# ounben/fishnet

Measured on AMD Instinct MI355X. Metric: NNUE evals/sec (node) at 1/2/4/8 MI355X + FT gather HBM GB/s as % of peak, higher is better.
Workload: dtype int16/int8

## Files before the change

fishnet_amd/csrc/gpu_nnue.hip:

```cpp
#include <stdarg.h>
#include <stdio.h>
#include <string.h>

#include <algorithm>
#include <atomic>
#include <chrono>
#include <condition_variable>
#include <memory>
#include <mutex>
#include <string>
#include <thread>
#include <vector>

#include "archive.h"
#include "host_board.h"
#include "kernels.h"
#include "sha256.h"

using namespace gn;

static thread_local std::string g_err;

static int fail(int code, const char *fmt, ...) {
  char buf[512];
// ... 116 lines not shown
    if (!r.u32(hs) || hs != ah) return fail(GN_E_FORMAT, "bad layer-stack hash in stack %d", s);
    bool ok = true;
    for (int i = 0; i < 16 && ok; ++i) ok = r.u32(reinterpret_cast<uint32_t &>(h.b0[s * 16 + i]));
    ok = ok && r.take(&h.w0[(size_t)s * 16 * l1], (size_t)16 * l1);
    for (int i = 0; i < 32 && ok; ++i) ok = r.u32(reinterpret_cast<uint32_t &>(h.b1[s * 32 + i]));
    ok = ok && r.take(&h.w1[s * 1024], 1024);
    ok = ok && r.u32(reinterpret_cast<uint32_t &>(h.b2[s]));
    ok = ok && r.take(&h.w2[s * 32], 32);
    if (!ok) return fail(GN_E_FORMAT, "truncated layer stack %d", s);
  }
  if (r.off != len) return fail(GN_E_FORMAT, "%zu trailing bytes after the network", len - r.off);
  return GN_OK;
}

template <class T>
struct DevBuf {
  T *p = nullptr;
  size_t cap = 0;
  hipError_t ensure(size_t n) {
    if (n <= cap) return hipSuccess;
    const size_t want = std::max(n, cap + cap / 2);
    if (p) (void)hipFree(p);
    p = nullptr;
    cap = 0;
    hipError_t e = hipMalloc(&p, (std::max<size_t>(want, 1) * sizeof(T) + 15) & ~(size_t)15);
    if (e == hipSuccess) cap = want;
    return e;
  }
  void release() {
    if (p) (void)hipFree(p);
    p = nullptr, cap = 0;
  }
};

struct EvalBufs {
  DevBuf<int2> osm, obg;
  DevBuf<uint8_t> nsm, nbg;
  void release() { osm.release(), obg.release(), nsm.release(), nbg.release(); }
};

constexpr size_t FAST_NB0 = 128, FAST_MAX = 4096;
struct FastBatch {
  size_t nb = 0, c1 = 0, c2 = 0;
  int mode = -1;
  uint64_t gen = 0;
  hipGraph_t graph = nullptr;
  hipGraphExec_t exec = nullptr;
  hipEvent_t done = nullptr;
  bool busy = false;
  gn_board *h_in = nullptr;
  gn_eval *h_out = nullptr;
  DevBuf<gn_board> all;
  DevBuf<gn_eval> rec;
  gn_board *in = nullptr, *r1 = nullptr, *r2 = nullptr;
  gn_eval *out = nullptr, *e1 = nullptr, *e2 = nullptr;
  DevBuf<uint64_t> off0, off1;
  DevBuf<uint16_t> m1, m2;
  DevBuf<int32_t> sv1, sv2;
  EvalBufs eb;
  ~FastBatch() {
    if (done) (void)hipEventDestroy(done);
    if (exec) (void)hipGraphExecDestroy(exec);
    if (graph) (void)hipGraphDestroy(graph);
    if (h_in) (void)hipHostFree(h_in);
    if (h_out) (void)hipHostFree(h_out);
    all.release(), rec.release();
    off0.release(), off1.release(), m1.release(), m2.release(), sv1.release(), sv2.release();
    eb.release();
  }
};

struct ExpSet {
  DevBuf<uint64_t> counts, offsets;
  DevBuf<uint32_t> owner;
  DevBuf<Board> unpacked;
  DevBuf<uint16_t> moves_tmp;
  const uint16_t *child_moves = nullptr;
  DevBuf<int2> pinfo;
  DevBuf<int2> p_osm, p_obg;
  DevBuf<uint8_t> p_nsm, p_nbg;
  EvalBufs eb;
  DevBuf<gn_board> children;
  int chain_k = 1;
  int slices = 1;
  bool planned = false;
  uint64_t etot = 0;
  void *scan_tmp = nullptr, *sort_tmp = nullptr;
  size_t scan_bytes = 0, sort_bytes = 0;
  hipEvent_t scored = nullptr;
  DevBuf<uint32_t> perr;
  DevBuf<unsigned long long> pstat;
  DevBuf<uint64_t> ent, eoff;
  DevBuf<TileDesc> tiles;
  DevBuf<uint32_t> btiles, border;
  void release() {
    perr.release(), pstat.release();
    ent.release(), eoff.release(), tiles.release(), btiles.release(), border.release();
    counts.release(), offsets.release(), owner.release(), unpacked.release(), moves_tmp.release();
    pinfo.release(), p_osm.release(), p_obg.release(), p_nsm.release(), p_nbg.release(), eb.release();
    children.release();
    if (scan_tmp) (void)hipFree(scan_tmp);
    if (sort_tmp) (void)hipFree(sort_tmp);
    scan_tmp = sort_tmp = nullptr, scan_bytes = sort_bytes = 0;
    if (scored) (void)hipEventDestroy(scored);
    scored = nullptr;
  }
};

struct Dev {
  int id = 0;
  hipStream_t stream = nullptr;
  void *net_mem[2] = {nullptr, nullptr};
  NetDevice net[2] = {};
  bool has[2] = {false, false};
  Tables *tables = nullptr;
  ExpSet cur, alt;
  DevBuf<gn_board> io_boards, frontier;
  DevBuf<gn_eval> io_out, io_out2;
  DevBuf<uint32_t> off32;
  DevBuf<uint16_t> moves;
  DevBuf<ChildDelta> deltas;
  DevBuf<uint64_t> kkeys, kkeys2;
  DevBuf<uint32_t> kidx, kperm;
  DevBuf<unsigned long long> sum;
  DevBuf<uint8_t> nslot;
  DevBuf<int32_t> part;
  bool part_locked = false;
  DevBuf<uint64_t> ebound;
  DevBuf<uint32_t> pool;
  DevBuf<uint16_t> bkeys, bkeys2;
  DevBuf<uint32_t> bidx;
  hipEvent_t done = nullptr;
  hipStream_t done_on = nullptr;
  float plan_ms = 0, stream_ms = 0, finish_ms = 0;
  struct ScoreLevel {
    DevBuf<uint64_t> sel, pos, counts, offsets;
    DevBuf<uint32_t> idx, owner;
    DevBuf<gn_board> boards, children;
    DevBuf<uint16_t> moves;
    DevBuf<gn_eval> ce;
    DevBuf<int32_t> sv;
    void release() {
      sel.release(), pos.release(), counts.release(), offsets.release(), idx.release(), owner.release();
      boards.release(), children.release(), moves.release(), ce.release(), sv.release();
    }
  } lv[2];
  hipStream_t copy = nullptr;
  hipEvent_t cev[2] = {nullptr, nullptr};
  DevBuf<gn_eval> po2[2], co2[2];
  DevBuf<gn_child> cc2[2];
  DevBuf<uint16_t> mv2[2];
  DevBuf<gn_board> roots, rboards, par;
  DevBuf<uint64_t> moff;
  DevBuf<uint16_t> codes, smoves;
  DevBuf<int32_t> rstatus;
  DevBuf<uint32_t> gidx;
  double t_upload = 0, t_replay = 0, t_compute = 0, t_download = 0, t_tail = 0;
  std::unique_ptr<FastBatch> fast[6][3][2];
  std::condition_variable fast_cv;
  hipStream_t front = nullptr;
  hipEvent_t ev_streamed = nullptr, ev_planned = nullptr;
  std::mutex mu;
};

static void swap_sets(Dev &d) { std::swap(d.cur, d.alt); }

static hipError_t seq_begin(Dev &d, hipStream_t s) {
  if (d.done_on && d.done_on != s) return hipStreamWaitEvent(s, d.done, 0);
  return hipSuccess;
}
static hipError_t seq_end(Dev &d, hipStream_t s) {
  hipError_t e = hipEventRecord(d.done, s);
  if (e == hipSuccess) d.done_on = s;
  return e;
}
static int check_plan(Dev &d, hipStream_t s) {
  if (!d.cur.planned || !d.cur.perr.p) return GN_OK;
  uint32_t e = 0;
  HIP_TRY(hipMemcpyAsync(&e, d.cur.perr.p, sizeof(e), hipMemcpyDeviceToHost, s));
  HIP_TRY(hipStreamSynchronize(s));
  if (e) return fail(GN_E_HIP, "planned expansion failed on the device (error bits 0x%x)", e);
  return GN_OK;
}

struct SeqGuard {
  Dev &d;
  hipStream_t s;
  hipError_t e;
  bool ended = false;
  SeqGuard(Dev &d_, hipStream_t s_) : d(d_), s(s_) { e = seq_begin(d, s); }
  hipError_t finish() {
    ended = true;
    hipError_t r = seq_end(d, s);
    return r == hipSuccess ? hipStreamSynchronize(s) : r;
  }
  ~SeqGuard() {
    if (!ended) (void)seq_end(d, s);
  }
};

#ifndef GN_MAX_LEADERS
#define GN_MAX_LEADERS 1
#endif
constexpr int MAX_LEADERS = GN_MAX_LEADERS;
struct BatchReq {
  const gn_board *boards;
  size_t n;
  int mode;
  gn_eval *out;
  int rc = GN_OK;
  bool done = false;
  bool taken = false;
  char err[256] = "";
};

struct gn_ctx {
  std::vector<std::unique_ptr<Dev>> devs;
  struct {
    std::mutex mu;
    std::condition_variable cv;
    std::vector<BatchReq *> q;
    int active = 0;
    uint64_t launches = 0, calls = 0;
  } co;
  bool coalesce = true;
  bool fast_batch = true;
  int pipeline = 2;
  std::atomic<uint64_t> graph_gen{0};
  std::atomic<uint64_t> fast_runs{0}, fast_fallbacks{0};
  gn_eval_params P;
  bool incremental = true;
  int swizzle = 9;
  int king_sort = 1;
  int chain = 81;
  bool king_cache = true;
  int stream_slices = 3;
  int64_t chunk_parents = 0;
  int l1[2] = {0, 0};
  uint32_t hash[2] = {0, 0};
  double t_parse = 0, t_total = 0;
};

enum { BIG = 0, SMALL = 1 };

static gn_eval_params default_params() {
  gn_eval_params P;
  P.small_net_threshold = 962;
  P.psqt_weight = 125;
  P.positional_weight = 131;
  P.reeval_threshold = 236;
  P.complexity_div_small = 18000;
  P.complexity_div_big = 18000;
  P.material_pawn_small = 535;
  P.material_pawn_big = 535;
  P.material_base = 77777;
  P.rule50_div = 212;
  P.value_clamp = 31506;
  const int32_t pv[5] = {208, 781, 825, 1276, 2538};
  memcpy(P.piece_value, pv, sizeof(pv));
  const double wa[4] = {-37.45051876, 121.19101539, -132.78783573, 420.70576692};
  memcpy(P.wdl_a, wa, sizeof(wa));
  P.wdl_material_min = 17;
  P.wdl_material_max = 78;
  P.wdl_material_anchor = 58;
  const int32_t ww[5] = {1, 3, 3, 5, 9};
  memcpy(P.wdl_piece_weight, ww, sizeof(ww));
  return P;
}

static size_t align256(size_t x) { return (x + 255) & ~(size_t)255; }

static int upload_net(Dev &d, int which, const HostNet &h) {
  const size_t RS = ft_row_stride((uint32_t)h.L1);
  size_t off[10], o = 0;
  const int carry = h.L1 == 128 ? 0 : CARRY_SLOTS;
  std::vector<int32_t> psqt((size_t)PSQT_BUCKETS * FT_ROWS);
  for (size_t r = 0; r < (size_t)FT_ROWS; ++r)
    for (int b = 0; b < PSQT_BUCKETS; ++b)
      memcpy(&psqt[(size_t)b * FT_ROWS + r], h.ft.data() + r * RS + 2 * (size_t)h.L1 + 4 * b, 4);
  const int KS = h.L1 / 64;
  std::vector<int8_t> w0f(h.w0.size());
  for (int b = 0; b < LAYER_STACKS; ++b)
    for (int ks = 0; ks < KS; ++ks)
      for (int ln = 0; ln < 64; ++ln)
        memcpy(&w0f[(((size_t)b * KS + ks) * 64 + ln) * 16],
               &h.w0[((size_t)b * 16 + (ln & 15)) * h.L1 + 64 * (size_t)ks + 16 * (ln >> 4)], 16);
  const size_t sz[10] = {((size_t)FT_ROWS + 4 * (size_t)carry + 128 * (size_t)carry + (carry ? 1 : 0)) * RS, h.bias.size() * 2, h.w0.size(), h.b0.size() * 4,
                         h.w1.size(), h.b1.size() * 4, h.w2.size(), h.b2.size() * 4, psqt.size() * 4, w0f.size()};
  const void *src[10] = {h.ft.data(), h.bias.data(), h.w0.data(), h.b0.data(),
                         h.w1.data(), h.b1.data(), h.w2.data(), h.b2.data(), psqt.data(), w0f.data()};
  for (int i = 0; i < 10; ++i) off[i] = o, o += align256(sz[i]);
  uint8_t *m = nullptr;
  if (hipMalloc(&m, o) != hipSuccess) return fail(GN_E_NOMEM, "device allocation of %zu bytes failed", o);
  d.net_mem[which] = m;
  for (int i = 0; i < 10; ++i)
    HIP_TRY(hipMemcpy(m + off[i], src[i], i == 0 ? (size_t)FT_ROWS * RS : sz[i], hipMemcpyHostToDevice));
  if (carry) HIP_TRY(hipMemset(m + off[0] + (size_t)FT_ROWS * RS, 0, 4 * (size_t)carry * RS));
  if (carry) HIP_TRY(hipMemset(m + off[0] + (size_t)ZERO_ROW * RS, 0, RS));
  NetDevice &n = d.net[which];
  n.L1 = h.L1;
  n.row_stride = (uint32_t)RS;
  n.carry_slots = carry;
  n.kc_slots = carry;
  n.ft = m + off[0];
  n.bias = reinterpret_cast<const int16_t *>(m + off[1]);
  n.w0 = reinterpret_cast<const int8_t *>(m + off[2]);
  n.b0 = reinterpret_cast<const int32_t *>(m + off[3]);
  n.w1 = reinterpret_cast<const int8_t *>(m + off[4]);
  n.b1 = reinterpret_cast<const int32_t *>(m + off[5]);
  n.w2 = reinterpret_cast<const int8_t *>(m + off[6]);
  n.b2 = reinterpret_cast<const int32_t *>(m + off[7]);
  n.psqt = reinterpret_cast<const int32_t *>(m + off[8]);
  n.w0f = reinterpret_cast<const int8_t *>(m + off[9]);
  d.has[which] = true;
  return GN_OK;
}

static void destroy(gn_ctx *ctx) {
  if (!ctx) return;
  for (auto &dp : ctx->devs) {
    Dev &d = *dp;
    (void)hipSetDevice(d.id);
    if (d.stream) (void)hipStreamSynchronize(d.stream);
    for (void *m : d.net_mem)
      if (m) (void)hipFree(m);
    if (d.tables) (void)hipFree(d.tables);
    d.cur.release(), d.alt.release();
    d.io_boards.release(), d.frontier.release(), d.io_out.release(), d.io_out2.release();
    d.off32.release(), d.moves.release(), d.sum.release(), d.deltas.release();
    d.part.release();
    if (d.front) (void)hipStreamSynchronize(d.front), (void)hipStreamDestroy(d.front);
    if (d.ev_streamed) (void)hipEventDestroy(d.ev_streamed);
    if (d.ev_planned) (void)hipEventDestroy(d.ev_planned);
    d.kkeys.release(), d.kkeys2.release(), d.kidx.release(), d.kperm.release();
    d.nslot.release();
    d.ebound.release(), d.pool.release();
    d.bkeys.release(), d.bkeys2.release(), d.bidx.release();
    d.lv[0].release(), d.lv[1].release();
    for (auto &row : d.fast)
      for (auto &pair : row)
        for (auto &f : pair) f.reset();
    for (int i = 0; i < 2; ++i) {
      d.po2[i].release(), d.co2[i].release(), d.cc2[i].release(), d.mv2[i].release();
      if (d.cev[i]) (void)hipEventDestroy(d.cev[i]);
    }
    d.roots.release(), d.rboards.release(), d.par.release(), d.moff.release(), d.codes.release();
    d.smoves.release(), d.rstatus.release(), d.gidx.release();
    if (d.copy) (void)hipStreamSynchronize(d.copy), (void)hipStreamDestroy(d.copy);
    if (d.done) (void)hipEventDestroy(d.done);
    if (d.stream) (void)hipStreamDestroy(d.stream);
  }
  delete ctx;
}

static int create(const uint8_t *big, size_t big_len, const uint8_t *small, size_t small_len, const int *devices,
                  int n_devices, gn_ctx **out) {
  if (!out) return fail(GN_E_INVALID, "out is NULL");
  *out = nullptr;
  if (!big && !small) return fail(GN_E_INVALID, "no network given");
  HostNet hn[2];
  if (big) {
    int rc = parse_net(big, big_len, hn[BIG]);
    if (rc) return rc;
  }
  if (small) {
    int rc = parse_net(small, small_len, hn[SMALL]);
    if (rc) return rc;
  }
  int count = 0;
  if (hipGetDeviceCount(&count) != hipSuccess || count <= 0) return fail(GN_E_NODEVICE, "no HIP device visible");
  std::vector<int> ids;
  if (devices && n_devices > 0) ids.assign(devices, devices + n_devices);
  else ids.push_back(0);
  std::unique_ptr<gn_ctx, void (*)(gn_ctx *)> ctx(new gn_ctx(), destroy);
  ctx->P = default_params();
  for (int w = 0; w < 2; ++w) ctx->l1[w] = hn[w].L1, ctx->hash[w] = hn[w].hash;
  for (int id : ids) {
    if (id < 0 || id >= count) return fail(GN_E_NODEVICE, "device %d out of range (%d visible)", id, count);
    hipDeviceProp_t prop;
    HIP_TRY(hipGetDeviceProperties(&prop, id));
    if (!strstr(prop.gcnArchName, "gfx950"))
      return fail(GN_E_NODEVICE, "device %d is %s; libgpu_nnue is built for gfx950 only", id, prop.gcnArchName);
    ctx->devs.emplace_back(new Dev());
    Dev &d = *ctx->devs.back();
    d.id = id;
    HIP_TRY(hipSetDevice(id));
    HIP_TRY(hipStreamCreateWithFlags(&d.stream, hipStreamNonBlocking));
    HIP_TRY(hipEventCreateWithFlags(&d.done, hipEventDisableTiming));
    HIP_TRY(hipStreamCreateWithFlags(&d.copy, hipStreamNonBlocking));
#ifdef GN_AB_FRONT_PRIORITY
    {
      int least = 0, greatest = 0;
      HIP_TRY(hipDeviceGetStreamPriorityRange(&least, &greatest));
      HIP_TRY(hipStreamCreateWithPriority(&d.front, hipStreamNonBlocking, greatest));
    }
#else
    HIP_TRY(hipStreamCreateWithFlags(&d.front, hipStreamNonBlocking));
#endif
    HIP_TRY(hipEventCreateWithFlags(&d.ev_streamed, hipEventDisableTiming));
    HIP_TRY(hipEventCreateWithFlags(&d.ev_planned, hipEventDisableTiming));
    for (int i = 0; i < 2; ++i) HIP_TRY(hipEventCreateWithFlags(&d.cev[i], hipEventDisableTiming));
#ifdef GN_AB_AUX_STREAMS
    {
      hipStream_t x[2];
      for (int i = 0; i < 2; ++i) HIP_TRY(hipStreamCreateWithFlags(&x[i], hipStreamNonBlocking));
    }
#endif
    HIP_TRY(hipMalloc(&d.tables, sizeof(Tables)));
    for (ExpSet *x : {&d.cur, &d.alt}) {
      HIP_TRY(x->perr.ensure(1));
      HIP_TRY(x->pstat.ensure(1));
      HIP_TRY(hipEventCreateWithFlags(&x->scored, hipEventDisableTiming));
    }
    HIP_TRY(hipMemset(d.alt.perr.p, 0, sizeof(uint32_t)));
    HIP_TRY(hipMemcpy(d.tables, &host_tables(), sizeof(Tables), hipMemcpyHostToDevice));
    for (int w = 0; w < 2; ++w)
      if (hn[w].L1) {
        int rc = upload_net(d, w, hn[w]);
        if (rc) return rc;
      }
// ... 61 lines not shown
                            mode == GN_MODE_FULL ? &P : nullptr, nsm.p, nbg.p));
  HIP_TRY(mark(2));
  if (mode != GN_MODE_SMALL)
    HIP_TRY(launch_eval_net(d.net[BIG], b, mode == GN_MODE_FULL ? nbg.p : nullptr, n, obg.p, perm, swz, s,
                            rows_out));
  HIP_TRY(mark(3));
  HIP_TRY(launch_finalize(b, n, mode, osm.p, obg.p, nsm.p, nbg.p, P, d.tables, out, s, score, counts));
  HIP_TRY(mark(4));
  return GN_OK;
}

static Dev *slot(gn_ctx *ctx, int s) {
  if (!ctx || s < 0 || s >= (int)ctx->devs.size()) return nullptr;
  return ctx->devs[s].get();
}

template <class F>
static void parallel_for(size_t n, size_t grain, F &&f) {
  unsigned hw = std::max(1u, std::min(16u, std::thread::hardware_concurrency()));
  size_t chunks = std::min<size_t>(hw, (n + grain - 1) / std::max<size_t>(grain, 1));
  if (chunks <= 1) {
    f(0, n);
    return;
  }
  std::vector<std::thread> th;
  size_t per = (n + chunks - 1) / chunks;
  for (size_t c = 0; c < chunks; ++c) {
    size_t lo = c * per, hi = std::min(n, lo + per);
    if (lo < hi) th.emplace_back([=, &f] { f(lo, hi); });
  }
  for (auto &t : th) t.join();
}

static int chain_len(const gn_ctx *ctx, Dev &d, size_t n) {
  if (!ctx->incremental || (ctx->chain >= -1 && ctx->chain <= 1) || !d.has[BIG] || !d.net[BIG].carry_slots)
    return 1;
  if (ctx->chain < 0) return -ctx->chain;
  size_t k = (size_t)ctx->chain;
  if ((n + k - 1) / k < 2048) k = std::max<size_t>(2, std::min(k, n / 2048));
  return (int)k;
}

static bool plan_path(const gn_ctx *ctx, const Dev &d, int mode) {
  return mode != GN_MODE_SMALL && ctx->incremental && d.has[BIG] &&
         (d.net[BIG].L1 == 3072 || d.net[BIG].L1 == 1024);
}

static int finalize_all(gn_ctx *ctx, Dev &d, const gn_board *parents, const gn_board *children, int mode,
                        gn_eval *parent_out, gn_eval *child_out, size_t n, size_t total, hipStream_t s,
                        bool score_parents, bool sliced = false) {
  const gn_eval_params &P = ctx->P;
  const ExpSet &x = d.cur;
  const SlicedOut sc = {&d.net[BIG], d.part.p, x.pinfo.p, (uint64_t)(n + total), (uint64_t)n},
                  sp = {&d.net[BIG], d.part.p, x.pinfo.p, (uint64_t)(n + total), 0};
  const bool fast = x.child_moves != nullptr;
  HIP_TRY(launch_finalize(children, total, mode, x.eb.osm.p, x.eb.obg.p, x.eb.nsm.p, x.eb.nbg.p, P, d.tables, child_out,
                          s, 0, nullptr, fast ? x.owner.p : nullptr, fast ? x.child_moves : nullptr,
                          fast ? x.unpacked.p : nullptr, sliced ? &sc : nullptr));
  if (parent_out)
    HIP_TRY(launch_finalize(parents, n, mode, x.p_osm.p, x.p_obg.p, x.p_nsm.p, x.p_nbg.p, P, d.tables, parent_out, s,
                            score_parents ? 1 : 0, x.counts.p, nullptr, nullptr, nullptr, sliced ? &sp : nullptr));
  return GN_OK;
}

static hipError_t count_children(Dev &d, const gn_board *parents, size_t n, hipStream_t s, size_t *total) {
  ExpSet &x = d.cur;
  hipError_t e;
  if ((e = x.counts.ensure(n + 1)) != hipSuccess || (e = x.offsets.ensure(n + 1)) != hipSuccess) return e;
  if ((e = hipMemsetAsync(x.counts.p + n, 0, sizeof(uint64_t), s)) != hipSuccess) return e;
  if ((e = launch_count_children(parents, n, d.tables, x.counts.p, s)) != hipSuccess) return e;
  if ((e = exclusive_scan_u64(x.counts.p, x.offsets.p, n + 1, x.scan_tmp, x.scan_bytes, s)) != hipSuccess) return e;
  uint64_t t = 0;
  if ((e = hipMemcpyAsync(&t, x.offsets.p + n, sizeof(t), hipMemcpyDeviceToHost, s)) != hipSuccess) return e;
  if ((e = hipStreamSynchronize(s)) != hipSuccess) return e;
  *total = (size_t)t;
  return hipSuccess;
}

struct GenOpts {
  hipEvent_t *ev = nullptr;
  unsigned long long *rows = nullptr;
  bool deltas = false;
  int chain_k = 1;
  bool plan = false;
  bool skip_internal = false;
  size_t limit = SIZE_MAX;
};
static int generate_children(Dev &d, const gn_board *parents, size_t n, gn_board *children_or_null, uint16_t *moves,
                             size_t *total, hipStream_t s, const GenOpts &o = {}) {
  ExpSet &x = d.cur;
  x.chain_k = o.deltas ? o.chain_k : 1;
  x.planned = o.deltas && o.plan;
  if (x.planned) {
    HIP_TRY(hipMemsetAsync(x.perr.p, 0, sizeof(uint32_t), s));
    HIP_TRY(hipMemsetAsync(x.pstat.p, 0, sizeof(unsigned long long), s));
  }
  if (x.chain_k > 1) HIP_TRY(d.nslot.ensure(n));
  HIP_TRY(x.counts.ensure(n + 1));
  HIP_TRY(x.offsets.ensure(n + 1));
  HIP_TRY(hipMemsetAsync(x.counts.p + n, 0, sizeof(uint64_t), s));
  if (x.planned) {
    HIP_TRY(d.ebound.ensure(n + 1));
    HIP_TRY(x.eoff.ensure(n + 1));
    HIP_TRY(hipMemsetAsync(d.ebound.p + n, 0, sizeof(uint64_t), s));
  }
  HIP_TRY(launch_count_children(parents, n, d.tables, x.counts.p, s, x.planned ? d.ebound.p : nullptr));
  HIP_TRY(exclusive_scan_u64(x.counts.p, x.offsets.p, n + 1, x.scan_tmp, x.scan_bytes, s));
  if (x.planned) HIP_TRY(exclusive_scan_u64(d.ebound.p, x.eoff.p, n + 1, x.scan_tmp, x.scan_bytes, s));
  if (o.ev) HIP_TRY(hipEventRecord(o.ev[0], s));
  uint64_t t = 0;
  HIP_TRY(hipMemcpyAsync(&t, x.offsets.p + n, sizeof(t), hipMemcpyDeviceToHost, s));
  if (x.planned) HIP_TRY(hipMemcpyAsync(&x.etot, x.eoff.p + n, sizeof(uint64_t), hipMemcpyDeviceToHost, s));
  HIP_TRY(hipStreamSynchronize(s));
  *total = (size_t)t;
  if (t > o.limit) return fail(GN_E_CAPACITY, "%zu children exceed capacity %zu", (size_t)t, o.limit);
  if (o.ev) HIP_TRY(hipEventRecord(o.ev[1], s));
  gn_board *children = children_or_null;
  const bool skip_boards = !children_or_null && x.planned && o.skip_internal;
  if (!children && !skip_boards) {
    HIP_TRY(x.children.ensure(std::max<size_t>(t, 1)));
    children = x.children.p;
  }
  if (o.deltas) HIP_TRY(d.deltas.ensure(std::max<size_t>(t, 1)));
  HIP_TRY(x.owner.ensure(std::max<size_t>(t, 1)));
  HIP_TRY(x.unpacked.ensure(std::max<size_t>(n, 1)));
  if (!moves) {
    HIP_TRY(x.moves_tmp.ensure(std::max<size_t>(t, 1)));
    moves = x.moves_tmp.p;
  }
  x.child_moves = moves;
  if (t) {
    HIP_TRY(launch_write_children(parents, n, d.tables, x.offsets.p, 0, t, children, moves, x.owner.p,
                                  o.deltas ? d.deltas.p : nullptr, x.chain_k > 1 ? d.nslot.p : nullptr, x.chain_k,
                                  o.rows, s, x.unpacked.p));
  }
  if (o.ev) HIP_TRY(hipEventRecord(o.ev[2], s));
  return GN_OK;
}

static GenOpts gen_opts(const gn_ctx *ctx, Dev &d, size_t n, int mode, size_t limit) {
  GenOpts g;
  g.deltas = ctx->incremental, g.chain_k = chain_len(ctx, d, n), g.plan = plan_path(ctx, d, mode);
  g.skip_internal = mode == GN_MODE_BIG, g.limit = limit;
  return g;
}

constexpr int EXP_FRONT = 1, EXP_BACK = 2;
struct EvalOpts {
  hipEvent_t *ev = nullptr;
  unsigned long long *rows = nullptr;
  bool score_parents = true;
  int phases = EXP_FRONT | EXP_BACK;
  hipEvent_t streamed = nullptr;
};
static int expand_evaluate(gn_ctx *ctx, Dev &d, const gn_board *parents, size_t n, const gn_board *children,
                           size_t total, int mode, gn_eval *parent_out, gn_eval *child_out, hipStream_t s,
                           const EvalOpts &o = {}) {
  if (mode < GN_MODE_FULL || mode > GN_MODE_SMALL) return fail(GN_E_INVALID, "bad mode %d", mode);
  if ((mode != GN_MODE_SMALL && !d.has[BIG]) || (mode != GN_MODE_BIG && !d.has[SMALL]))
    return fail(GN_E_NONET, "mode %d needs a network that is not loaded", mode);
  ExpSet &x = d.cur;
  hipEvent_t *const ev = o.ev;
  const int phases = o.phases;
  if (!ctx->incremental) {
    if (!(phases & EXP_BACK)) return GN_OK;
    if (total) {
      int rc = evaluate_on(ctx, d, children, total, mode, child_out, s, nullptr, nullptr, 0);
      if (rc) return rc;
    }
    return parent_out ? evaluate_on(ctx, d, parents, n, mode, parent_out, s, nullptr, nullptr, o.score_parents ? 1 : 0,
                                    x.counts.p)
                      : GN_OK;
  }
  auto mark = [&](int k) -> hipError_t { return ev ? hipEventRecord(ev[k], s) : hipSuccess; };
  const gn_eval_params &P = ctx->P;
  const uint64_t *off = x.offsets.p;
  const ChildDelta *dl = d.deltas.p;
  const bool f = mode == GN_MODE_FULL;
  const size_t K = (size_t)std::max(1, x.chain_k), nblk = (n + K - 1) / K;
  const bool ordered = ctx->king_sort && nblk > 1;
  auto plan_args = [&] {
    PlanStreamArgs a;
    a.parents = parents, a.n = n, a.offsets = off, a.deltas = dl;
    a.need_parent = f ? x.p_nbg.p : nullptr, a.need_child = f ? x.eb.nbg.p : nullptr;
    a.out_parent = x.p_obg.p, a.out_child = x.eb.obg.p;
    a.next_slot = x.chain_k > 1 ? d.nslot.p : nullptr, a.chain_k = x.chain_k, a.kc = ctx->king_cache ? 1 : 0;
    a.eoff = x.eoff.p, a.ent = x.ent.p, a.tiles = x.tiles.p, a.btiles = x.btiles.p;
    a.pool = d.pool.p, a.err = x.perr.p, a.rows_out = o.rows, a.pads_out = x.pstat.p;
    a.slices = x.slices, a.npos = n + total;
    if (x.slices > 1) a.part = d.part.p, a.pinfo = x.pinfo.p;
    return a;
  };
  if (phases & EXP_FRONT) {
    const size_t nt = std::max<size_t>(total, 1);
    if (mode != GN_MODE_BIG) {
      HIP_TRY(x.eb.osm.ensure(nt));
      HIP_TRY(x.p_osm.ensure(n));
    }
    if (mode != GN_MODE_SMALL) {
      HIP_TRY(x.eb.obg.ensure(nt));
      HIP_TRY(x.p_obg.ensure(n));
    }
    if (f) {
      HIP_TRY(x.eb.nsm.ensure(nt));
      HIP_TRY(x.eb.nbg.ensure(nt));
      HIP_TRY(x.p_nsm.ensure(n));
      HIP_TRY(x.p_nbg.ensure(n));
      HIP_TRY(launch_classify(parents, n, P, x.p_nsm.p, x.p_nbg.p, s));
      HIP_TRY(launch_classify(children, total, P, x.eb.nsm.p, x.eb.nbg.p, s));
    }
    HIP_TRY(mark(0));
    if (mode != GN_MODE_BIG) {
      HIP_TRY(launch_expand_net(d.net[SMALL], parents, n, off, children, dl, f ? x.p_nsm.p : nullptr,
                                f ? x.eb.nsm.p : nullptr, x.p_osm.p, x.eb.osm.p, ctx->swizzle & 1, s));
      if (f) {
        HIP_TRY(launch_reeval(x.p_osm.p, x.p_nsm.p, n, P, x.p_nbg.p, s));
        HIP_TRY(launch_reeval(x.eb.osm.p, x.eb.nsm.p, total, P, x.eb.nbg.p, s));
      }
    }
    HIP_TRY(mark(1));
    x.slices = 1;
    if (mode != GN_MODE_SMALL && x.planned) {
      HIP_TRY(x.ent.ensure(x.etot + (size_t)ENT_SPARE * (nblk + 1)));
      HIP_TRY(x.tiles.ensure((n + total) / 16 + (K + 2) * nblk + 2));
      HIP_TRY(x.btiles.ensure(nblk + 1));
      HIP_TRY(d.pool.ensure(88));
      if (d.net[BIG].L1 == 3072 && ctx->stream_slices == 3) {
        const size_t need = (size_t)GN_PART_SLICES * 16 * (n + total);
        bool ok = d.part_locked ? d.part.cap >= need : d.part.ensure(need) == hipSuccess;
        ok = ok && x.pinfo.ensure(n + total) == hipSuccess;
        if (ok) x.slices = 3;
        else {
          (void)hipGetLastError();
          if (!d.part_locked) d.part.release();
          x.pinfo.release();
        }
      }
      if (ordered) {
        HIP_TRY(d.bkeys.ensure(nblk));
        HIP_TRY(d.bkeys2.ensure(nblk));
        HIP_TRY(d.bidx.ensure(nblk));
        HIP_TRY(x.border.ensure(nblk));
        HIP_TRY(block_order(parents, n, (uint32_t)K, (uint32_t)nblk, d.bkeys.p, d.bidx.p, d.bkeys2.p, x.border.p,
                            x.sort_tmp, x.sort_bytes, s));
      }
      PlanStreamArgs a = plan_args();
      a.mid = ev ? ev[4] : nullptr;
      HIP_TRY(launch_plan_stream(d.net[BIG], a, PLAN_PHASE, s));
    }
  }
  if (!(phases & EXP_BACK)) return GN_OK;
  bool fused = false;
  if (mode != GN_MODE_SMALL) {
    if (x.planned) {
      HIP_TRY(hipMemsetAsync(d.pool.p, 0, 88 * sizeof(uint32_t), s));
#ifndef GN_AB_FINISH_SEPARATE
      fused = x.slices > 1;
#endif
      if (ev && (phases & EXP_FRONT) == 0) HIP_TRY(hipEventRecord(ev[7], s));
      PlanStreamArgs a = plan_args();
      a.swz = (ctx->swizzle >> 2) & 1 ? 1 : (ctx->swizzle >> 3) & 1 ? 2 : 0;
      a.order = ordered ? x.border.p : nullptr;
      a.fin = ev ? ev[6] : nullptr, a.streamed = o.streamed, a.finish = !fused;
      HIP_TRY(launch_plan_stream(d.net[BIG], a, STREAM_PHASE, s));
    } else {
      HIP_TRY(launch_expand_net(d.net[BIG], parents, n, off, children, dl, f ? x.p_nbg.p : nullptr,
                                f ? x.eb.nbg.p : nullptr, x.p_obg.p, x.eb.obg.p, ctx->swizzle & 1, s));
    }
  }
  HIP_TRY(mark(2));
  int rc = finalize_all(ctx, d, parents, children, mode, parent_out, child_out, n, total, s, o.score_parents, fused);
  if (rc) return rc;
  HIP_TRY(mark(3));
  return GN_OK;
}

struct Replies {
  const gn_eval *rec;
  const uint16_t *moves;
};
static int resolve_scores(gn_ctx *ctx, Dev &d, const gn_board *boards, size_t n, int mode, gn_eval *out,
                          int32_t *sv_out, hipStream_t s, int depth = 2, const Replies *replies = nullptr) {
  if (!n || depth <= 0 || !out) return GN_OK;
  Dev::ScoreLevel &L = d.lv[2 - depth];
  HIP_TRY(L.sel.ensure(n + 1));
  HIP_TRY(L.pos.ensure(n + 1));
  HIP_TRY(launch_score_select(out, n, L.sel.p, s));
  HIP_TRY(exclusive_scan_u64(L.sel.p, L.pos.p, n + 1, d.cur.scan_tmp, d.cur.scan_bytes, s));
  uint64_t m = 0;
  HIP_TRY(hipMemcpyAsync(&m, L.pos.p + n, sizeof(m), hipMemcpyDeviceToHost, s));
  HIP_TRY(hipStreamSynchronize(s));
  if (!m) return GN_OK;
  HIP_TRY(L.idx.ensure(m));
  HIP_TRY(L.boards.ensure(m));
  HIP_TRY(L.counts.ensure(m + 1));
  HIP_TRY(L.offsets.ensure(m + 1));
  HIP_TRY(launch_score_gather(boards, L.sel.p, L.pos.p, n, L.idx.p, L.boards.p, s));
  if (replies) {
    uint64_t t = 0;
    HIP_TRY(launch_score_replies(L.idx.p, m, d.cur.offsets.p, L.counts.p, L.offsets.p, d.cur.scan_tmp,
                                 d.cur.scan_bytes, &t, s));
    HIP_TRY(L.moves.ensure(std::max<uint64_t>(t, 1)));
    HIP_TRY(L.children.ensure(std::max<uint64_t>(t, 1)));
    HIP_TRY(L.ce.ensure(std::max<uint64_t>(t, 1)));
    HIP_TRY(L.sv.ensure(std::max<uint64_t>(t, 1)));
    HIP_TRY(launch_score_replies_fill(L.idx.p, m, d.cur.offsets.p, L.offsets.p, replies->rec, replies->moves,
                                      d.cur.unpacked.p, d.tables, L.ce.p, L.children.p, L.moves.p, s));
    int rc = resolve_scores(ctx, d, L.children.p, t, mode, L.ce.p, L.sv.p, s, depth - 1);
    if (rc) return rc;
    HIP_TRY(launch_score_reduce(L.boards.p, m, L.idx.p, L.offsets.p, L.moves.p, L.ce.p, L.sv.p, ctx->P, out, sv_out,
                                s));
    return GN_OK;
  }
  HIP_TRY(hipMemsetAsync(L.counts.p + m, 0, sizeof(uint64_t), s));
  HIP_TRY(launch_count_children(L.boards.p, m, d.tables, L.counts.p, s));
  HIP_TRY(exclusive_scan_u64(L.counts.p, L.offsets.p, m + 1, d.cur.scan_tmp, d.cur.scan_bytes, s));
  uint64_t t = 0;
  HIP_TRY(hipMemcpyAsync(&t, L.offsets.p + m, sizeof(t), hipMemcpyDeviceToHost, s));
  HIP_TRY(hipStreamSynchronize(s));
  HIP_TRY(L.moves.ensure(std::max<uint64_t>(t, 1)));
  HIP_TRY(L.owner.ensure(std::max<uint64_t>(t, 1)));
  HIP_TRY(L.children.ensure(std::max<uint64_t>(t, 1)));
  HIP_TRY(L.ce.ensure(std::max<uint64_t>(t, 1)));
  HIP_TRY(L.sv.ensure(std::max<uint64_t>(t, 1)));
  HIP_TRY(launch_write_children(L.boards.p, m, d.tables, L.offsets.p, 0, t, L.children.p, L.moves.p, L.owner.p,
                                nullptr, nullptr, 1, nullptr, s));
  int rc = evaluate_on(ctx, d, L.children.p, t, mode, L.ce.p, s, nullptr);
  if (rc) return rc;
  if ((rc = resolve_scores(ctx, d, L.children.p, t, mode, L.ce.p, L.sv.p, s, depth - 1)) != GN_OK) return rc;
  HIP_TRY(launch_score_reduce(L.boards.p, m, L.idx.p, L.offsets.p, L.moves.p, L.ce.p, L.sv.p, ctx->P, out, sv_out, s));
  return GN_OK;
}

static void partition(const uint32_t *weights, size_t n, int ns, size_t *bounds) {
  uint64_t total = 0;
  for (size_t i = 0; i < n; ++i) total += weights ? weights[i] : 1u;
  bounds[0] = 0;
  size_t i = 0;
  uint64_t acc = 0;
  for (int k = 1; k < ns; ++k) {
    const uint64_t target = (total * (uint64_t)k + (uint64_t)ns - 1) / (uint64_t)ns;
    while (i < n && acc < target) acc += weights ? weights[i++] : (++i, 1u);
    bounds[k] = i;
  }
  bounds[ns] = n;
}

template <class F>
static int for_each_device(gn_ctx *ctx, F &&f) {
  const size_t nd = ctx->devs.size();
  std::vector<int> rcs(nd, GN_OK);
  std::vector<std::string> errs(nd);
  auto work = [&](size_t k) {
    Dev &d = *ctx->devs[k];
    std::lock_guard<std::mutex> lk(d.mu);
    rcs[k] = f(k, d);
    if (rcs[k]) errs[k] = g_err;
  };
  if (nd == 1) work(0);
  else {
    std::vector<std::thread> th;
    for (size_t k = 0; k < nd; ++k) th.emplace_back(work, k);
    for (auto &t : th) t.join();
  }
  for (size_t k = 0; k < nd; ++k)
    if (rcs[k]) {
      g_err = errs[k];
      return rcs[k];
    }
  return GN_OK;
}

static int fast_build(gn_ctx *ctx, Dev &d, FastBatch &f, size_t nb, int mode) {
  f.nb = nb, f.c1 = nb / 2 + 256, f.c2 = nb / 4 + 256, f.mode = mode, f.gen = ctx->graph_gen.load();
  const size_t na = nb + f.c1 + f.c2;
  HIP_TRY(hipEventCreateWithFlags(&f.done, hipEventDisableTiming));
  HIP_TRY(hipHostMalloc((void **)&f.h_in, nb * sizeof(gn_board), hipHostMallocDefault));
  HIP_TRY(hipHostMalloc((void **)&f.h_out, (nb + 1) * sizeof(gn_eval), hipHostMallocDefault));
  HIP_TRY(f.all.ensure(na));
  HIP_TRY(f.rec.ensure(na + 1));
  f.in = f.all.p, f.r1 = f.in + nb, f.r2 = f.r1 + f.c1;
  f.out = f.rec.p + 1, f.e1 = f.out + nb, f.e2 = f.e1 + f.c1;
  HIP_TRY(f.m1.ensure(f.c1));
  HIP_TRY(f.sv1.ensure(f.c1));
  HIP_TRY(f.m2.ensure(f.c2));
  HIP_TRY(f.sv2.ensure(f.c2));
  HIP_TRY(f.off0.ensure(nb + 1));
  HIP_TRY(f.off1.ensure(f.c1 + 1));
  HIP_TRY(f.eb.osm.ensure(na));
  HIP_TRY(f.eb.obg.ensure(na));
  HIP_TRY(f.eb.nsm.ensure(na));
  HIP_TRY(f.eb.nbg.ensure(na));
  const hipStream_t s = d.stream;
  uint32_t *flag = reinterpret_cast<uint32_t *>(f.rec.p);
  HIP_TRY(hipStreamBeginCapture(s, hipStreamCaptureModeThreadLocal));
  auto seq = [&]() -> int {
    HIP_TRY(hipMemcpyAsync(f.in, f.h_in, nb * sizeof(gn_board), hipMemcpyHostToDevice, s));
    HIP_TRY(launch_reply_level(f.in, nb, d.tables, f.off0.p, f.c1, f.r1, f.m1.p, flag, 1, s));
    HIP_TRY(launch_reply_level(f.r1, f.c1, d.tables, f.off1.p, f.c2, f.r2, f.m2.p, flag, 0, s));
    int rc = evaluate_on(ctx, d, f.all.p, na, mode, f.out, s, nullptr, nullptr, 1, nullptr, &f.eb, false);
    if (rc) return rc;
#ifndef GN_AB_FAST_TWO_REDUCES
    HIP_TRY(launch_score_reduce2(f.r1, f.c1, f.off1.p, f.m2.p, f.e2, f.sv2.p, f.e1, f.sv1.p, f.in, nb, f.off0.p, f.m1.p,
                                 ctx->P, f.out, s));
#else
    HIP_TRY(launch_score_reduce(f.r1, f.c1, nullptr, f.off1.p, f.m2.p, f.e2, f.sv2.p, ctx->P, f.e1, f.sv1.p, s));
    HIP_TRY(launch_score_reduce(f.in, nb, nullptr, f.off0.p, f.m1.p, f.e1, f.sv1.p, ctx->P, f.out, nullptr, s));
#endif
    HIP_TRY(hipMemcpyAsync(f.h_out, f.rec.p, (nb + 1) * sizeof(gn_eval), hipMemcpyDeviceToHost, s));
// ... 1383 lines not shown
    acc += ms / (float)iters;
    return e;
  };
  float stage[8] = {0, 0, 0, 0, 0, 0, 0, 0}, pl = 0, st = 0, fi = 0;
  for (int it = 0; it < iters; ++it) {
    const size_t o = 2 + (size_t)NE * it;
    for (int k = 0; k < 8 && stage_ms; ++k)
      if (pipe && k == 5) {
        HIP_TRY(add_ms(stage[k], o + 5, o + 8));
        HIP_TRY(add_ms(stage[k], o + 11, o + 6));
      } else {
        HIP_TRY(add_ms(stage[k], o + k, o + (k < 7 ? k + 1 : 9)));
      }
    if (!d->cur.planned) continue;
    HIP_TRY(add_ms(pl, o + 5, o + 8));
    HIP_TRY(add_ms(st, o + (pipe ? 11 : 8), o + 10));
    HIP_TRY(add_ms(fi, o + 10, o + 6));
  }
  if (stage_ms) std::copy(stage, stage + 8, stage_ms);
  if (d->cur.planned) d->plan_ms = pl, d->stream_ms = st, d->finish_ms = fi;
  if ((rc = check_plan(*d, s)) != GN_OK) return rc;
  if (pipe) {
    swap_sets(*d);
    rc = check_plan(*d, s);
    swap_sets(*d);
    if (rc) return rc;
  }
  if (ft_rows) {
    unsigned long long r[2] = {0, 0};
    HIP_TRY(hipMemcpy(r, d->sum.p, sizeof(r), hipMemcpyDeviceToHost));
    *ft_rows = ctx->incremental ? (r[1] ? r[1] : r[0]) : 0;
  }
  return GN_OK;
}

int gn_checksum_device(gn_ctx *ctx, int device_slot, const void *d_ptr, size_t bytes, uint64_t *sum) {
  Dev *d = slot(ctx, device_slot);
  if (!d || !sum || (bytes && !d_ptr)) return fail(GN_E_INVALID, "bad argument");
  std::lock_guard<std::mutex> lk(d->mu);
  HIP_TRY(hipSetDevice(d->id));
  SeqGuard sg(*d, d->stream);
  HIP_TRY(sg.e);
  HIP_TRY(d->sum.ensure(2));
  HIP_TRY(hipMemsetAsync(d->sum.p, 0, sizeof(unsigned long long), d->stream));
  HIP_TRY(launch_checksum(d_ptr, bytes, d->sum.p, d->stream));
  unsigned long long r = 0;
  HIP_TRY(hipMemcpyAsync(&r, d->sum.p, sizeof(r), hipMemcpyDeviceToHost, d->stream));
  HIP_TRY(hipStreamSynchronize(d->stream));
  *sum = r;
  return GN_OK;
}

int gn_random_games_device(gn_ctx *ctx, int device_slot, uint64_t seed, size_t first_game, size_t n_games, int plies,
                           gn_board *d_out, void *stream) {
  Dev *d = slot(ctx, device_slot);
  if (!d) return fail(GN_E_INVALID, "bad context or device slot");
  if (n_games && !d_out) return fail(GN_E_INVALID, "NULL buffer");
  if (plies < 0 || plies > 1000) return fail(GN_E_INVALID, "plies out of range");
  std::lock_guard<std::mutex> lk(d->mu);
  HIP_TRY(hipSetDevice(d->id));
  SeqGuard sg(*d, stream ? (hipStream_t)stream : d->stream);
  HIP_TRY(sg.e);
  HIP_TRY(launch_random_games(seed, first_game, n_games, plies, d->tables, d_out, sg.s));
  return GN_OK;
}

int gn_set_option(gn_ctx *ctx, int option, int64_t value) {
  if (!ctx) return fail(GN_E_INVALID, "ctx is NULL");
  ++ctx->graph_gen;
  switch (option) {
  case GN_OPT_INCREMENTAL_CHILDREN:
    ctx->incremental = value != 0;
    return GN_OK;
  case GN_OPT_XCD_SWIZZLE:
    ctx->swizzle = (int)(value & 15);
    return GN_OK;
  case GN_OPT_KING_SORT:
    if (value < 0 || value > 2) return fail(GN_E_INVALID, "king sort must be 0, 1 or 2");
    ctx->king_sort = (int)value;
    return GN_OK;
  case GN_OPT_KING_CACHE:
    ctx->king_cache = value != 0;
    return GN_OK;
  case GN_OPT_CHAIN:
    if (value < -(1 << 20) || value > (1 << 20)) return fail(GN_E_INVALID, "chain length out of range");
    ctx->chain = (int)value;
    return GN_OK;
  case GN_OPT_STREAM_SLICES:
    if (value != 1 && value != 3) return fail(GN_E_INVALID, "stream slices must be 1 or 3");
    ctx->stream_slices = (int)value;
    return GN_OK;
  case GN_OPT_CHUNK_PARENTS:
    if (value < 0) return fail(GN_E_INVALID, "chunk size < 0");
    ctx->chunk_parents = value;
    return GN_OK;
  case GN_OPT_COALESCE:
    ctx->coalesce = value != 0;
    return GN_OK;
  case GN_OPT_FAST_BATCH:
    ctx->fast_batch = value != 0;
    return GN_OK;
  case GN_OPT_EXPAND_PIPELINE:
    if (value < 0 || value > 2) return fail(GN_E_INVALID, "GN_OPT_EXPAND_PIPELINE %lld not in 0..2", (long long)value);
    ctx->pipeline = (int)value;
    return GN_OK;
  default:
    return fail(GN_E_INVALID, "unknown option %d", option);
  }
}

int gn_get_option(const gn_ctx *ctx, int option, int64_t *value) {
  if (!ctx || !value) return fail(GN_E_INVALID, "NULL argument");
  switch (option) {
  case GN_OPT_INCREMENTAL_CHILDREN:
    *value = ctx->incremental;
    return GN_OK;
  case GN_OPT_XCD_SWIZZLE:
    *value = ctx->swizzle;
    return GN_OK;
  case GN_OPT_KING_SORT:
    *value = ctx->king_sort;
    return GN_OK;
  case GN_OPT_KING_CACHE:
    *value = ctx->king_cache;
    return GN_OK;
  case GN_OPT_CHAIN:
    *value = ctx->chain;
    return GN_OK;
  case GN_OPT_STREAM_SLICES:
    *value = ctx->stream_slices;
    return GN_OK;
  case GN_OPT_CHUNK_PARENTS:
    *value = ctx->chunk_parents;
    return GN_OK;
  case GN_OPT_COALESCE:
    *value = ctx->coalesce;
    return GN_OK;
  case GN_OPT_FAST_BATCH:
    *value = ctx->fast_batch;
    return GN_OK;
  case GN_OPT_EXPAND_PIPELINE:
    *value = ctx->pipeline;
    return GN_OK;
  case GN_STAT_FAST_BATCHES:
    *value = (int64_t)ctx->fast_runs.load();
    return GN_OK;
  case GN_STAT_FAST_FALLBACKS:
    *value = (int64_t)ctx->fast_fallbacks.load();
    return GN_OK;
  case GN_STAT_BATCH_LAUNCHES:
  case GN_STAT_BATCH_CALLS: {
    auto &C = const_cast<gn_ctx *>(ctx)->co;
    std::lock_guard<std::mutex> lk(C.mu);
    *value = (int64_t)(option == GN_STAT_BATCH_LAUNCHES ? C.launches : C.calls);
    return GN_OK;
  }
  case GN_STAT_PLAN_NS:
  case GN_STAT_STREAM_NS:
  case GN_STAT_FINISH_NS: {
    float m = 0;
    for (auto &dp : ctx->devs)
      m = std::max(m, option == GN_STAT_PLAN_NS     ? dp->plan_ms
                      : option == GN_STAT_STREAM_NS ? dp->stream_ms
                                                    : dp->finish_ms);
    *value = (int64_t)((double)m * 1e6);
    return GN_OK;
  }
  case GN_STAT_HOST_PARSE_NS:
  case GN_STAT_HOST_TOTAL_NS:
    *value = (int64_t)((option == GN_STAT_HOST_PARSE_NS ? ctx->t_parse : ctx->t_total) * 1e6);
    return GN_OK;
  case GN_STAT_HOST_UPLOAD_NS:
  case GN_STAT_HOST_REPLAY_NS:
  case GN_STAT_HOST_COMPUTE_NS:
  case GN_STAT_HOST_DOWNLOAD_NS:
  case GN_STAT_HOST_TAIL_NS: {
    double m = 0;
    for (auto &dp : ctx->devs) {
      const Dev &d = *dp;
      m = std::max(m, option == GN_STAT_HOST_UPLOAD_NS    ? d.t_upload
                      : option == GN_STAT_HOST_REPLAY_NS  ? d.t_replay
                      : option == GN_STAT_HOST_COMPUTE_NS ? d.t_compute
                      : option == GN_STAT_HOST_DOWNLOAD_NS ? d.t_download
                                                           : d.t_tail);
    }
    *value = (int64_t)(m * 1e6);
    return GN_OK;
  }
  case GN_STAT_SCRATCH_PADS: {
    int64_t sum = 0;
    for (auto &dp : ctx->devs) {
      Dev &d = *dp;
      std::lock_guard<std::mutex> lk(d.mu);
      if (!d.cur.pstat.p) continue;
      HIP_TRY(hipSetDevice(d.id));
      if (d.done_on) HIP_TRY(hipEventSynchronize(d.done));
      unsigned long long v = 0;
      HIP_TRY(hipMemcpy(&v, d.cur.pstat.p, sizeof(v), hipMemcpyDeviceToHost));
      sum += (int64_t)v;
    }
    *value = sum;
    return GN_OK;
  }
  default:
    return fail(GN_E_INVALID, "unknown option %d", option);
  }
}

// ... 66 lines not shown
```

fishnet_amd/csrc/kernels.h:

```cpp
#pragma once
#include <hip/hip_runtime.h>
#include <stddef.h>
#include <stdint.h>

#include "nnue.h"

#ifndef GN_RING
#define GN_RING 4
#endif
#ifndef GN_SLICE_RING
#define GN_SLICE_RING 4
#endif
#ifndef GN_SCR_GAP
#define GN_SCR_GAP (GN_RING > GN_SLICE_RING ? GN_RING : GN_SLICE_RING)
#endif
#ifndef GN_FRONT_WG
#define GN_FRONT_WG 128
#endif
static_assert(GN_FRONT_WG == 64 || GN_FRONT_WG == 128 || GN_FRONT_WG == 256, "front workgroups of 1, 2 or 4 waves");

constexpr unsigned ENT_SPARE = 32;

#ifdef GN_PART_INPLACE
#define GN_PART_SLICES 1
#else
#define GN_PART_SLICES 3
#endif

namespace gn {

hipError_t launch_eval_net(const NetDevice &net, const gn_board *boards, const uint8_t *need, size_t n,
                           int2 *out, const uint32_t *perm, int swz, hipStream_t s,
                           unsigned long long *rows_out = nullptr, const gn_eval_params *cls = nullptr,
                           uint8_t *need_small = nullptr, uint8_t *need_big = nullptr);
hipError_t launch_checksum(const void *p, size_t bytes, unsigned long long *out, hipStream_t s);
hipError_t block_order(const gn_board *parents, size_t n, uint32_t K, uint32_t nblk, uint16_t *keys, uint32_t *idx,
                       uint16_t *keys_out, uint32_t *order, void *&temp, size_t &temp_bytes, hipStream_t s);
hipError_t king_sort(const gn_board *boards, size_t n, uint64_t *keys, uint32_t *idx, uint64_t *keys_out,
                     uint32_t *perm, bool placement, void *&temp, size_t &temp_bytes, hipStream_t s);
hipError_t launch_expand_net(const NetDevice &net, const gn_board *parents, size_t n, const uint64_t *offsets,
                             const gn_board *children, const ChildDelta *deltas, const uint8_t *need_parent,
                             const uint8_t *need_child, int2 *out_parent, int2 *out_child, int swz, hipStream_t s);
struct TileDesc {
  uint32_t e_end[2];
  uint32_t p_first;
  uint32_t first;
  uint8_t meta[16];
  int32_t psq[16][2];
  int16_t adj[16];
};
static_assert(sizeof(TileDesc) == 192, "TileDesc is 192 bytes");
constexpr int PLAN_PHASE = 1, STREAM_PHASE = 2;
struct PlanStreamArgs {
  const gn_board *parents = nullptr;
  size_t n = 0;
  const uint64_t *offsets = nullptr;
  const ChildDelta *deltas = nullptr;
  const uint8_t *need_parent = nullptr, *need_child = nullptr;
  int2 *out_parent = nullptr, *out_child = nullptr;
  const uint8_t *next_slot = nullptr;
  int chain_k = 1;
  int kc = 0;
  const uint64_t *eoff = nullptr;
  uint64_t *ent = nullptr;
  TileDesc *tiles = nullptr;
  uint32_t *btiles = nullptr;
  uint32_t *pool = nullptr;
  uint32_t *err = nullptr;
  unsigned long long *rows_out = nullptr;
  unsigned long long *pads_out = nullptr;
  const uint32_t *order = nullptr;
  int slices = 1;
  int32_t *part = nullptr;
  size_t npos = 0;
  int2 *pinfo = nullptr;
  bool finish = true;
  int swz = 0;
  hipEvent_t mid = nullptr;
  hipEvent_t fin = nullptr, streamed = nullptr;
};
hipError_t launch_plan_stream(const NetDevice &net, const PlanStreamArgs &a, int phases, hipStream_t s);
hipError_t launch_classify(const gn_board *boards, size_t n, const gn_eval_params &P, uint8_t *need_small,
                           uint8_t *need_big, hipStream_t s);
hipError_t launch_reeval(const int2 *out_small, const uint8_t *need_small, size_t n, const gn_eval_params &P,
                         uint8_t *need_big, hipStream_t s);
struct SlicedOut {
  const NetDevice *net;
  const int32_t *part;
  const int2 *pinfo;
  uint64_t npos, qoff;
};
hipError_t launch_finalize(const gn_board *boards, size_t n, int mode, const int2 *out_small,
                           const int2 *out_big, const uint8_t *need_small, const uint8_t *need_big,
                           const gn_eval_params &P, const Tables *tables, gn_eval *out, hipStream_t s,
                           int score, const uint64_t *counts = nullptr, const uint32_t *owner = nullptr,
                           const uint16_t *moves = nullptr, const Board *unpacked = nullptr,
                           const SlicedOut *sliced = nullptr);
hipError_t launch_score_select(const gn_eval *out, size_t n, uint64_t *sel, hipStream_t s);
hipError_t launch_score_gather(const gn_board *boards, const uint64_t *sel, const uint64_t *pos, size_t n,
                               uint32_t *idx, gn_board *sb, hipStream_t s);
hipError_t launch_score_replies(const uint32_t *idx, size_t m, const uint64_t *off, uint64_t *counts,
                                uint64_t *coff, void *&temp, size_t &temp_bytes, uint64_t *total_host, hipStream_t s);
hipError_t launch_score_replies_fill(const uint32_t *idx, size_t m, const uint64_t *off, const uint64_t *coff,
                                     const gn_eval *rec, const uint16_t *moves, const Board *unpacked,
                                     const Tables *tables, gn_eval *ce, gn_board *cb, uint16_t *cm, hipStream_t s);
hipError_t launch_score_reduce(const gn_board *sb, size_t m, const uint32_t *idx, const uint64_t *off,
                               const uint16_t *moves, const gn_eval *ce, const int32_t *csv, const gn_eval_params &P,
                               gn_eval *out, int32_t *sv, hipStream_t s);
hipError_t launch_score_reduce2(const gn_board *sb1, size_t m1, const uint64_t *off1, const uint16_t *moves2,
                                const gn_eval *ce2, const int32_t *csv2, gn_eval *out1, int32_t *sv1,
                                const gn_board *sb0, size_t m0, const uint64_t *off0, const uint16_t *moves1,
                                const gn_eval_params &P, gn_eval *out0, hipStream_t s);
hipError_t launch_reply_level(const gn_board *boards, size_t n, const Tables *tables, uint64_t *off, size_t cap,
                              gn_board *rb, uint16_t *rm, uint32_t *flag, int first, hipStream_t s);
hipError_t launch_count_children(const gn_board *boards, size_t n, const Tables *tables, uint64_t *counts,
                                 hipStream_t s, uint64_t *ebound = nullptr);
hipError_t launch_write_children(const gn_board *boards, size_t n, const Tables *tables, const uint64_t *offsets,
                                 size_t c0, size_t nc, gn_board *children, uint16_t *moves, uint32_t *owner,
                                 ChildDelta *deltas, uint8_t *next_slot, int chain_k, unsigned long long *rows,
                                 hipStream_t s, Board *unpacked = nullptr);
hipError_t launch_count_sum(const gn_board *boards, size_t n, const Tables *tables,
                            unsigned long long *total, hipStream_t s);
hipError_t launch_random_positions(uint64_t seed, size_t first, size_t n, int max_plies, const Tables *tables,
                                   gn_board *out, hipStream_t s);
hipError_t launch_random_games(uint64_t seed, size_t first_game, size_t n_games, int plies, const Tables *tables,
                               gn_board *out, hipStream_t s);
hipError_t launch_replay_games(const gn_board *roots, size_t ng, const uint64_t *moff, const uint16_t *codes,
                               const Tables *tables, gn_board *boards, uint16_t *smoves, int32_t *status, hipStream_t s);
hipError_t launch_gather_boards(const gn_board *src, const uint32_t *idx, size_t n, gn_board *dst, hipStream_t s);
hipError_t launch_pack_children(const gn_eval *in, size_t n, gn_child *out, hipStream_t s);
hipError_t launch_offsets_u32(const uint64_t *in, size_t n, uint32_t *out, hipStream_t s);
hipError_t exclusive_scan_u64(const uint64_t *counts, uint64_t *offsets, size_t n1, void *&temp,
                              size_t &temp_bytes, hipStream_t s);

}
```

fishnet_amd/csrc/kernels.hip:

```cpp
#include <stdio.h>
#include <stdlib.h>
#include <string.h>

#include <algorithm>

#include <hipcub/hipcub.hpp>

#include "device_util.h"
#include "kernels.h"

#ifndef GN_SMALL_DEPTH
#define GN_SMALL_DEPTH 4
#endif
#ifndef GN_SMALL_WPE
#define GN_SMALL_WPE 8
#endif


namespace gn {

constexpr int LS_SCRATCH = 16 * 16 * 4 + 16 * 32 + 16 * 4;

template <int L1, int NW, class Valid, class Emit>
__device__ __forceinline__ void layer_stack_tile(const NetDevice &net, const uint8_t *xt, uint8_t *ls,
// ... 976 lines not shown
          rm[r] = m;
        }
        ++r;
      });
    }
    base += cnt;
  }
  const uint32_t lim = total < cap ? total : cap;
#pragma unroll 1
  for (uint32_t r = t; r < lim; r += NT) {
    uint32_t u = 0;
#pragma unroll
    for (uint32_t step = NT / 2; step; step >>= 1)
      if (part[u + step - 1] <= r) u += step;
    const uint32_t cu = part[u] - (u ? part[u - 1] : 0u);
    if (cu > MAXM) continue;
    const uint32_t k = r - (part[u] - cu);
    const uint16_t m = smv[u][k];
    Board B;
    unpack(boards[u * q + spos[u][k]], B);
    pack(do_move(B, m, nullptr), rb[r]);
    rm[r] = m;
  }
  if (t == 0) {
    off[n] = total < cap ? total : cap;
    if (first) *flag = total > cap ? 1u : 0u;
    else if (total > cap) atomicOr(flag, 1u);
  }
  for (uint32_t r = total + t; r < cap; r += NT) rb[r] = gn_board{};
}

hipError_t launch_reply_level(const gn_board *boards, size_t n, const Tables *tables, uint64_t *off, size_t cap,
                              gn_board *rb, uint16_t *rm, uint32_t *flag, int first, hipStream_t s) {
  if (!n || n > 16384 || cap >= 0x80000000ull) return hipErrorInvalidValue;
  hipLaunchKernelGGL(reply_level_kernel, dim3(1), dim3(GN_RL_THREADS), 0, s, boards, (uint32_t)n, tables, off,
                     (uint32_t)cap, rb, rm, flag, first);
  return hipGetLastError();
}

hipError_t launch_score_reduce2(const gn_board *sb1, size_t m1, const uint64_t *off1, const uint16_t *moves2,
                                const gn_eval *ce2, const int32_t *csv2, gn_eval *out1, int32_t *sv1,
                                const gn_board *sb0, size_t m0, const uint64_t *off0, const uint16_t *moves1,
                                const gn_eval_params &P, gn_eval *out0, hipStream_t s) {
  const ReduceLevel a = {sb1, m1, off1, moves2, ce2, csv2, out1, sv1}, b = {sb0, m0, off0, moves1, out1, sv1, out0, nullptr};
  hipLaunchKernelGGL(score_reduce2_kernel, dim3(1), dim3(1024), 0, s, a, b, P);
  return hipGetLastError();
}

hipError_t launch_score_reduce(const gn_board *sb, size_t m, const uint32_t *idx, const uint64_t *off,
                               const uint16_t *moves, const gn_eval *ce, const int32_t *csv, const gn_eval_params &P,
                               gn_eval *out, int32_t *sv, hipStream_t s) {
  if (!m) return hipSuccess;
  hipLaunchKernelGGL(score_reduce_kernel, dim3(blocks_for(m, 256)), dim3(256), 0, s, sb, m, idx, off, moves, ce, csv,
                     P, out, sv);
  return hipGetLastError();
}

__global__ void count_children_kernel(const gn_board *__restrict__ boards, size_t n, const Tables *__restrict__ tables,
                                      uint64_t *__restrict__ counts, uint64_t *__restrict__ ebound) {
  __shared__ Tables T;
  load_tables(T, tables);
  const size_t i = (size_t)blockIdx.x * blockDim.x + threadIdx.x;
  if (i >= n) return;
  Board B;
  uint64_t c = 0, kmoves = 0;
  if (unpack(boards[i], B)) {
    const Bitboard king = B.byType[KING] & color_bb(B, B.stm);
    gen_legal(B, T, [&](uint16_t m) {
      ++c;
      kmoves += (sqbb(move_from(m)) & king) != 0;
    });
  }
  counts[i] = c;
  if (ebound) {
    const uint64_t P = popcnt(B.byType[0]);
    ebound[i] = c || P ? 2 * (P + 2) + 2 * GN_SCR_GAP + 8 * (c - kmoves) + (P + 6 + GN_SCR_GAP) * kmoves +
                             6 * ((c + 1) / 16 + 2)
                       : 0;
  }
}

__global__ void child_moves_kernel(const gn_board *__restrict__ boards, size_t n, const Tables *__restrict__ tables,
                                   const uint64_t *__restrict__ offsets, uint16_t *__restrict__ moves,
                                   uint32_t *__restrict__ owner, uint8_t *__restrict__ next_slot, int chain_k,
                                   unsigned long long *__restrict__ rows, Board *__restrict__ unpacked) {
  __shared__ Tables T;
  load_tables(T, tables);
  const size_t i = (size_t)blockIdx.x * blockDim.x + threadIdx.x;
  if (i >= n) return;
  uint32_t slot = 255;
  Board B;
  if (!unpack(boards[i], B)) {
    if (next_slot) next_slot[i] = 255;
    return;
  }
  if (unpacked) unpacked[i] = B;
  Board N;
  Bitboard S = 0;
  if (next_slot && i + 1 < n) {
    const gn_board nb = boards[i + 1];
    const int pn = popcnt(nb.occ);
    if (pn >= 2 && pn <= 32) {
      unpack(nb, N);
      S = (B.byColor[0] ^ N.byColor[0]) | (B.byColor[1] ^ N.byColor[1]) | (B.byType[0] ^ N.byType[0]);
#pragma unroll
      for (int t = PAWN; t <= KING; ++t) S |= B.byType[t] ^ N.byType[t];
    }
  }
  const int us = B.stm;
  const Bitboard occ = B.byType[0];
  const uint64_t k0 = offsets[i];
  uint64_t k = k0;
  gen_legal(B, T, [&](uint16_t m) {
    moves[k] = m;
    owner[k] = (uint32_t)i;
    if (S) {
      const int from = move_from(m), to = move_to(m), type = move_type(m);
      Bitboard sm, cocc;
      int kto = to, rto = to;
      if (type == MT_CASTLING) {
        const int kside = to > from;
        kto = rel_sq(us, kside ? 6 : 2), rto = rel_sq(us, kside ? 5 : 3);
        sm = (kto != from ? sqbb(from) | sqbb(kto) : 0) | (rto != to ? sqbb(to) | sqbb(rto) : 0);
        cocc = (occ ^ sqbb(from) ^ sqbb(to)) | sqbb(kto) | sqbb(rto);
      } else {
        const int capsq = type == MT_EN_PASSANT ? to - (us == WHITE ? 8 : -8) : to;
        sm = sqbb(from) | sqbb(to) | sqbb(capsq);
        cocc = (occ & ~(sqbb(from) | sqbb(capsq))) | sqbb(to);
      }
      if (sm == S && cocc == N.byType[0]) {
        bool same;
        if (type == MT_CASTLING)
          same = (N.byType[KING] & N.byColor[us] & sqbb(kto)) && (N.byType[ROOK] & N.byColor[us] & sqbb(rto));
        else
          same = piece_on(N, to) ==
                 (type == MT_PROMOTION ? make_piece(us, move_promo(m)) : piece_on(B, from));
        if (same) slot = (uint32_t)(k - k0);
      }
    }
    ++k;
  });
  if (next_slot) next_slot[i] = (uint8_t)slot;
  if (rows) {
    unsigned long long r = 2ull * popcnt(occ);
    if (slot != 255 && chain_k > 1 && (i + 1) % (size_t)chain_k != 0) r -= 2ull * popcnt(N.byType[0]) - 2;
    atomicAdd(rows, r);
  }
}

__global__ void child_boards_kernel(const gn_board *__restrict__ boards, size_t c0, size_t nc,
                                    const uint16_t *__restrict__ moves, const uint32_t *__restrict__ owner,
                                    gn_board *__restrict__ children, ChildDelta *__restrict__ deltas,
                                    unsigned long long *__restrict__ rows, const Board *__restrict__ unpacked) {
  const size_t c = c0 + (size_t)blockIdx.x * blockDim.x + threadIdx.x;
  unsigned long long nr = 0;
  if (c < c0 + nc) {
    const uint32_t i = owner[c];
    Board B;
    if (unpacked) B = unpacked[i];
    else unpack(boards[i], B);
    Dirty d;
    const Board C = do_move(B, moves[c], &d);
    if (children) pack(C, children[c]);
    if (deltas) deltas[c] = make_child_delta(B, C, d);
    nr = d.king_moved ? popcnt(C.byType[0]) + d.n_rem + d.n_add : 2 * (d.n_rem + d.n_add);
  }
  if (rows) {
    __shared__ unsigned long long part[GN_FRONT_WG / 64];
#pragma unroll
    for (int off = 32; off; off >>= 1) nr += __shfl_down(nr, off, 64);
    if ((threadIdx.x & 63) == 0) part[threadIdx.x >> 6] = nr;
    __syncthreads();
    if (threadIdx.x == 0) {
      unsigned long long t = 0;
#pragma unroll
      for (int w = 0; w < GN_FRONT_WG / 64; ++w) t += part[w];
      atomicAdd(rows, t);
    }
  }
}

__global__ void count_sum_kernel(const gn_board *__restrict__ boards, size_t n, const Tables *__restrict__ tables,
                                 unsigned long long *__restrict__ total) {
  __shared__ Tables T;
  __shared__ unsigned long long part[4];
  load_tables(T, tables);
  const size_t i = (size_t)blockIdx.x * blockDim.x + threadIdx.x;
  unsigned long long c = 0;
  if (i < n) {
    Board B;
    if (unpack(boards[i], B)) gen_legal(B, T, [&](uint16_t) { ++c; });
  }
  for (int off = 32; off; off >>= 1) c += __shfl_down(c, off, 64);
  if ((threadIdx.x & 63) == 0) part[threadIdx.x >> 6] = c;
  __syncthreads();
  if (threadIdx.x == 0) {
    unsigned long long s = 0;
    for (int w = 0; w < (int)(blockDim.x >> 6); ++w) s += part[w];
    if (s) atomicAdd(total, s);
  }
}

__global__ void random_positions_kernel(uint64_t seed, size_t first, size_t n, int max_plies,
                                        const Tables *__restrict__ tables, gn_board *__restrict__ out) {
  __shared__ Tables T;
  load_tables(T, tables);
  const size_t i = (size_t)blockIdx.x * blockDim.x + threadIdx.x;
  if (i >= n) return;
  gn_board pb;
  pack(random_playout(seed + first + i, max_plies, T), pb);
  out[i] = pb;
}

__global__ void random_games_kernel(uint64_t seed, size_t first_game, size_t n_games, int plies,
                                    const Tables *__restrict__ tables, gn_board *__restrict__ out) {
  __shared__ Tables T;
  load_tables(T, tables);
  const size_t g = (size_t)blockIdx.x * blockDim.x + threadIdx.x;
  if (g >= n_games) return;
  gn_board *dst = out + g * (size_t)(plies + 1);
  random_game(seed + first_game + g, plies, T, [&](int k, const Board &B, uint16_t) {
    gn_board pb;
    pack(B, pb);
    dst[k] = pb;
  });
}

__global__ void replay_games_kernel(const gn_board *__restrict__ roots, size_t ng, const uint64_t *__restrict__ moff,
// ... 30 lines not shown
  const size_t i = (size_t)blockIdx.x * blockDim.x + threadIdx.x;
  if (i < n) dst[i] = src[idx[i]];
}

template <class Key>
__global__ void king_keys_kernel(const gn_board *__restrict__ boards, size_t n, Key *__restrict__ keys,
                                 uint32_t *__restrict__ idx, int bkt) {
  const size_t i = (size_t)blockIdx.x * blockDim.x + threadIdx.x;
  if (i >= n) return;
  const gn_board p = boards[i];
  uint64_t wlo, whi;
  piece_words(p, wlo, whi);
  uint64_t o = p.occ;
  int wk = 64, bk = 64;
  uint64_t home = 0;
  const int c = popcnt(o) <= 32 ? popcnt(o) : 0;
  for (int k = 0; k < c; ++k) {
    const int s = pop_lsb(o), pc = piece_nibble(wlo, whi, k);
    if (pc == make_piece(WHITE, KING)) wk = s;
    if (pc == make_piece(BLACK, KING)) bk = s;
    const int r = s >> 3, f = s & 7;
    constexpr int BACK[8] = {ROOK, KNIGHT, BISHOP, QUEEN, KING, BISHOP, KNIGHT, ROOK};
    const int want = r == 0 ? make_piece(WHITE, BACK[f]) : r == 1 ? make_piece(WHITE, PAWN)
                   : r == 6 ? make_piece(BLACK, PAWN) : r == 7 ? make_piece(BLACK, BACK[f]) : -1;
    if (pc == want) home |= 1ull << s;
  }
  const uint32_t b = c ? (uint32_t)(c - 1) / 4 : 0;
  if constexpr (sizeof(Key) == 2) {
    keys[i] = (Key)(wk < 64 && bk < 64 ? ((bkt ? b << 12 : 0u) | (uint32_t)(wk << 6 | bk)) : 0xFFFF);
    idx[i] = (uint32_t)i;
    return;
  }
  uint64_t key = ~0ull;
  if (wk < 64 && bk < 64) {
    const uint64_t lo16 = home & 0xFFFF, hi16 = home >> 48;
    const uint64_t h30 = (lo16 & 0xF) | ((lo16 >> 1) & ~0xFull)
                         | ((hi16 & 0xFFF) | ((hi16 >> 1) & ~0xFFFull)) << 15;
    uint64_t r = 0, t = h30;
    for (int k = 0; k < 30; ++k, t >>= 1) r = r << 1 | (t & 1);
    key = bkt ? (uint64_t)wk << 58 | (uint64_t)bk << 52 | (uint64_t)b << 49 | r << 19
              : (uint64_t)wk << 58 | (uint64_t)bk << 52 | r << 22;
  }
  keys[i] = (Key)key;
  idx[i] = (uint32_t)i;
}

__global__ void checksum_kernel(const uint8_t *__restrict__ p, size_t bytes, unsigned long long *__restrict__ out) {
  const size_t nw = (bytes + 7) / 8;
  unsigned long long acc = 0;
  for (size_t i = (size_t)blockIdx.x * blockDim.x + threadIdx.x; i < nw; i += (size_t)gridDim.x * blockDim.x) {
    uint64_t w = 0;
    if (8 * i + 8 <= bytes) w = *reinterpret_cast<const uint64_t *>(p + 8 * i);
    else
      for (size_t k = 8 * i; k < bytes; ++k) w |= (uint64_t)p[k] << (8 * (k - 8 * i));
    acc += Xoshiro::mix(w ^ (i * 0x9E3779B97F4A7C15ull));
  }
  for (int off = 32; off; off >>= 1) acc += __shfl_down(acc, off, 64);
  if ((threadIdx.x & 63) == 0 && acc) atomicAdd(out, acc);
}

hipError_t launch_checksum(const void *p, size_t bytes, unsigned long long *out, hipStream_t s) {
  if (!bytes) return hipSuccess;
  const size_t nw = (bytes + 7) / 8;
  const unsigned g = (unsigned)std::min<size_t>(8192, (nw + 255) / 256);
  hipLaunchKernelGGL(checksum_kernel, dim3(g), dim3(256), 0, s, (const uint8_t *)p, bytes, out);
  return hipGetLastError();
}

__global__ void offsets_u32_kernel(const uint64_t *__restrict__ in, size_t n, uint32_t *__restrict__ out) {
  const size_t i = (size_t)blockIdx.x * blockDim.x + threadIdx.x;
  if (i < n) out[i] = (uint32_t)in[i];
}

hipError_t launch_count_children(const gn_board *boards, size_t n, const Tables *tables, uint64_t *counts,
                                 hipStream_t s, uint64_t *ebound) {
  if (!n) return hipSuccess;
  hipLaunchKernelGGL(count_children_kernel, dim3(blocks_for(n, GN_FRONT_WG)), dim3(GN_FRONT_WG), 0, s, boards, n, tables, counts,
                     ebound);
  return hipGetLastError();
}

hipError_t launch_write_children(const gn_board *boards, size_t n, const Tables *tables, const uint64_t *offsets,
                                 size_t c0, size_t nc, gn_board *children, uint16_t *moves, uint32_t *owner,
                                 ChildDelta *deltas, uint8_t *next_slot, int chain_k, unsigned long long *rows,
                                 hipStream_t s, Board *unpacked) {
  if (!n) return hipSuccess;
  if (!moves || !owner) return hipErrorInvalidValue;
  hipLaunchKernelGGL(child_moves_kernel, dim3(blocks_for(n, GN_FRONT_WG)), dim3(GN_FRONT_WG), 0, s, boards, n, tables, offsets, moves,
                     owner, next_slot, chain_k, rows, unpacked);
  if (nc)
    hipLaunchKernelGGL(child_boards_kernel, dim3(blocks_for(nc, GN_FRONT_WG)), dim3(GN_FRONT_WG), 0, s, boards, c0, nc, moves, owner,
                       children, deltas, rows, unpacked);
  return hipGetLastError();
}

hipError_t launch_count_sum(const gn_board *boards, size_t n, const Tables *tables, unsigned long long *total,
                            hipStream_t s) {
  if (!n) return hipSuccess;
  hipLaunchKernelGGL(count_sum_kernel, dim3(blocks_for(n, 256)), dim3(256), 0, s, boards, n, tables, total);
  return hipGetLastError();
}

hipError_t launch_random_positions(uint64_t seed, size_t first, size_t n, int max_plies, const Tables *tables,
                                   gn_board *out, hipStream_t s) {
  if (!n) return hipSuccess;
  hipLaunchKernelGGL(random_positions_kernel, dim3(blocks_for(n, 128)), dim3(128), 0, s, seed, first, n, max_plies,
                     tables, out);
  return hipGetLastError();
}

hipError_t launch_random_games(uint64_t seed, size_t first_game, size_t n_games, int plies, const Tables *tables,
                               gn_board *out, hipStream_t s) {
  if (!n_games) return hipSuccess;
  hipLaunchKernelGGL(random_games_kernel, dim3(blocks_for(n_games, 128)), dim3(128), 0, s, seed, first_game, n_games,
                     plies, tables, out);
  return hipGetLastError();
}

hipError_t launch_replay_games(const gn_board *roots, size_t ng, const uint64_t *moff, const uint16_t *codes,
                               const Tables *tables, gn_board *boards, uint16_t *smoves, int32_t *status, hipStream_t s) {
  if (!ng) return hipSuccess;
  hipLaunchKernelGGL(replay_games_kernel, dim3(blocks_for(ng, 64)), dim3(64), 0, s, roots, ng, moff, codes, tables,
                     boards, smoves, status);
  return hipGetLastError();
}

hipError_t launch_gather_boards(const gn_board *src, const uint32_t *idx, size_t n, gn_board *dst, hipStream_t s) {
  if (!n) return hipSuccess;
  hipLaunchKernelGGL(gather_boards_kernel, dim3(blocks_for(n, 256)), dim3(256), 0, s, src, idx, n, dst);
  return hipGetLastError();
}

hipError_t launch_offsets_u32(const uint64_t *in, size_t n, uint32_t *out, hipStream_t s) {
  if (!n) return hipSuccess;
  hipLaunchKernelGGL(offsets_u32_kernel, dim3(blocks_for(n, 256)), dim3(256), 0, s, in, n, out);
  return hipGetLastError();
}

template <class Key>
static hipError_t king_sort_t(const gn_board *boards, size_t n, Key *keys, uint32_t *idx, Key *keys_out,
                              uint32_t *perm, void *&temp, size_t &temp_bytes, hipStream_t s) {
  constexpr int bkt = 1;
  hipLaunchKernelGGL(king_keys_kernel<Key>, dim3(blocks_for(n, 256)), dim3(256), 0, s, boards, n, keys, idx, bkt);
  hipError_t e = hipGetLastError();
  if (e != hipSuccess) return e;
  constexpr int BITS = 8 * sizeof(Key);
  size_t need = 0;
  e = hipcub::DeviceRadixSort::SortPairs(nullptr, need, keys, keys_out, idx, perm, (int)n, 0, BITS, s);
  if (e != hipSuccess) return e;
  if (need > temp_bytes) {
    if (temp) (void)hipFree(temp);
    temp = nullptr;
    temp_bytes = 0;
    if ((e = hipMalloc(&temp, need)) != hipSuccess) return e;
    temp_bytes = need;
  }
  return hipcub::DeviceRadixSort::SortPairs(temp, temp_bytes, keys, keys_out, idx, perm, (int)n, 0, BITS, s);
}

hipError_t king_sort(const gn_board *boards, size_t n, uint64_t *keys, uint32_t *idx, uint64_t *keys_out,
                     uint32_t *perm, bool placement, void *&temp, size_t &temp_bytes, hipStream_t s) {
  if (!n) return hipSuccess;
  if (placement) return king_sort_t(boards, n, keys, idx, keys_out, perm, temp, temp_bytes, s);
  return king_sort_t(boards, n, reinterpret_cast<uint16_t *>(keys), idx, reinterpret_cast<uint16_t *>(keys_out), perm,
                     temp, temp_bytes, s);
}

__global__ void block_keys_kernel(const gn_board *__restrict__ parents, size_t n, uint32_t K, uint32_t nblk,
                                  uint16_t *__restrict__ keys, uint32_t *__restrict__ idx) {
  const uint32_t b = blockIdx.x * blockDim.x + threadIdx.x;
  if (b >= nblk) return;
  const size_t pb = (size_t)b * K, pe = pb + K < n ? pb + K : n;
  const gn_board p = parents[pb + (pe - pb) / 2];
  uint64_t wlo, whi;
  piece_words(p, wlo, whi);
  uint64_t o = p.occ;
  int wk = 63, bk = 63;
  const int c = popcnt(o) <= 32 ? popcnt(o) : 0;
  for (int k = 0; k < c; ++k) {
    const int sq = pop_lsb(o), pc = piece_nibble(wlo, whi, k);
    if (pc == make_piece(WHITE, KING)) wk = sq;
    if (pc == make_piece(BLACK, KING)) bk = sq;
  }
  keys[b] = (uint16_t)(wk << 6 | bk);
  idx[b] = b;
}

hipError_t block_order(const gn_board *parents, size_t n, uint32_t K, uint32_t nblk, uint16_t *keys, uint32_t *idx,
                       uint16_t *keys_out, uint32_t *order, void *&temp, size_t &temp_bytes, hipStream_t s) {
  if (!nblk) return hipSuccess;
  hipLaunchKernelGGL(block_keys_kernel, dim3(blocks_for(nblk, GN_FRONT_WG)), dim3(GN_FRONT_WG), 0, s, parents, n, K, nblk, keys, idx);
  hipError_t e = hipGetLastError();
  if (e != hipSuccess) return e;
  size_t need = 0;
  e = hipcub::DeviceRadixSort::SortPairs(nullptr, need, keys, keys_out, idx, order, (int)nblk, 0, 12, s);
  if (e != hipSuccess) return e;
  if (need > temp_bytes) {
    if (temp) (void)hipFree(temp);
    temp = nullptr;
    temp_bytes = 0;
    if ((e = hipMalloc(&temp, need)) != hipSuccess) return e;
    temp_bytes = need;
  }
  return hipcub::DeviceRadixSort::SortPairs(temp, temp_bytes, keys, keys_out, idx, order, (int)nblk, 0, 12, s);
}

hipError_t exclusive_scan_u64(const uint64_t *counts, uint64_t *offsets, size_t n1, void *&temp, size_t &temp_bytes,
                              hipStream_t s) {
  size_t need = 0;
  hipError_t e = hipcub::DeviceScan::ExclusiveSum(nullptr, need, counts, offsets, n1, s);
  if (e != hipSuccess) return e;
  if (need > temp_bytes) {
    if (temp) (void)hipFree(temp);
    temp = nullptr;
    temp_bytes = 0;
    if ((e = hipMalloc(&temp, need)) != hipSuccess) return e;
    temp_bytes = need;
  }
  return hipcub::DeviceScan::ExclusiveSum(temp, temp_bytes, counts, offsets, n1, s);
}

hipError_t launch_expand_net(const NetDevice &net, const gn_board *parents, size_t n, const uint64_t *offsets,
                             const gn_board *children, const ChildDelta *deltas, const uint8_t *need_parent,
                             const uint8_t *need_child, int2 *out_parent, int2 *out_child, int swz, hipStream_t s) {
  if (!n) return hipSuccess;
  if (n >= 0x80000000ull) return hipErrorInvalidValue;
  if (net.L1 != 128) return hipErrorInvalidValue;
  const unsigned g = (unsigned)(swz ? 8 * ((n + 7) / 8) : n);
  hipLaunchKernelGGL((expand_eval_kernel<128, 16>), dim3(g), dim3(256), 0, s, net, parents, offsets, children, deltas,
                     need_parent, need_child, out_parent, out_child, n, swz);
  return hipGetLastError();
}

}
```

fishnet_amd/csrc/nnue.h:

```cpp
#pragma once
#include <stdint.h>

#include "chess.h"

namespace gn {

constexpr int FT_INPUTS = 22528;
constexpr int FT_BIAS_ROW = FT_INPUTS;
constexpr int FT_ROWS = FT_INPUTS + 1;
#ifndef GN_ROW_ALIGN
#define GN_ROW_ALIGN 128
#endif
constexpr uint32_t ft_row_stride(uint32_t l1) { return (2 * l1 + 32 + GN_ROW_ALIGN - 1) / GN_ROW_ALIGN * GN_ROW_ALIGN; }
constexpr int CARRY_SLOTS = 2048;
constexpr int CARRY_ROW0 = FT_ROWS;
constexpr int KC_ROW0 = CARRY_ROW0 + 4 * CARRY_SLOTS;
static_assert(KC_ROW0 + 128 * CARRY_SLOTS <= (1 << 19), "carry and king-cache rows must fit the 19-bit row field");
constexpr int SCR_ROWS = 130;
constexpr int POOL_PER_XCD = 256;
constexpr int SCR_SLOTS = 8 * POOL_PER_XCD;
static_assert(SCR_ROWS * SCR_SLOTS <= 132 * CARRY_SLOTS, "scratch slots fit the rows behind the FT rows");
constexpr int ZERO_ROW = FT_ROWS + 132 * CARRY_SLOTS;
static_assert(ZERO_ROW < (1 << 19), "the zero row fits the 19-bit row field");
constexpr int PSQT_BUCKETS = 8;
constexpr int LAYER_STACKS = 8;
constexpr uint32_t NNUE_VERSION = 0x7AF32F20u;

struct NetDevice {
  int L1;
  uint32_t row_stride;
  int carry_slots;
  int kc_slots;
  const uint8_t *ft;
  const int16_t *bias;
  const int8_t *w0;
  const int32_t *b0;
  const int8_t *w1;
  const int32_t *b1;
  const int8_t *w2;
  const int32_t *b2;
  const int32_t *psqt;
  const int8_t *w0f;
};

GN_HD int feature_index(int persp, int sq, int pc, int ksq) {
  const int kf = ksq & 7;
  const int orient = (kf < 4 ? 7 : 0) ^ (persp ? 56 : 0);
  const int rel_rank = (ksq >> 3) ^ (persp ? 7 : 0);
  const int bucket = 4 * (7 - rel_rank) + (kf < 4 ? kf : 7 - kf);
  const int pt = pc & 7;
  const int plane = pt == KING ? 10 : 2 * (pt - 1) + ((pc >> 3) != persp);
  return (sq ^ orient) + 64 * plane + 704 * bucket;
}

struct ChildDelta {
  uint16_t idx[2][4];
  uint32_t meta;
  uint32_t pad;
};
static_assert(sizeof(ChildDelta) == 24, "ChildDelta is 24 bytes");

GN_HD ChildDelta make_child_delta(const Board &parent, const Board &child, const Dirty &d) {
  ChildDelta cd;
  uint32_t meta = 0;
#pragma unroll
  for (int h = 0; h < 2; ++h) {
    const int ksq = king_square(child, h);
    cd.idx[h][0] = cd.idx[h][1] = cd.idx[h][2] = cd.idx[h][3] = 0;
    if (d.king_moved && h == parent.stm) {
      meta |= 1u << (8 + h);
      const bool castle = d.n_add == 2;
      cd.idx[h][0] = (uint16_t)d.rem_sq[0];
      cd.idx[h][1] = (uint16_t)d.add_sq[0];
      cd.idx[h][2] = (uint16_t)(castle ? d.rem_sq[1] : 64);
      cd.idx[h][3] = (uint16_t)(castle ? d.add_sq[1] : 64);
    } else {
      cd.idx[h][0] = (uint16_t)feature_index(h, d.rem_sq[0], d.rem_pc[0], ksq);
      if (d.n_rem > 1) cd.idx[h][1] = (uint16_t)feature_index(h, d.rem_sq[1], d.rem_pc[1], ksq);
      cd.idx[h][2] = (uint16_t)feature_index(h, d.add_sq[0], d.add_pc[0], ksq);
      if (d.n_add > 1) cd.idx[h][3] = (uint16_t)feature_index(h, d.add_sq[1], d.add_pc[1], ksq);
      meta |= (uint32_t)(d.n_rem | (d.n_add << 2)) << (4 * h);
    }
  }
  meta |= (uint32_t)child.stm << 10;
  meta |= (uint32_t)((popcnt(child.byType[0]) - 1) / 4) << 11;
  meta |= (uint32_t)popcnt(child.byType[0]) << 14;
  cd.meta = meta;
  cd.pad = 0;
  return cd;
}

GN_HD int packed_features(const gn_board &p, uint16_t *rows_white, uint16_t *rows_black) {
  uint64_t wlo, whi;
  piece_words(p, wlo, whi);
  const int c = popcnt(p.occ);
  int wk = -1, bk = -1;
  bool ok = c >= 2 && c <= 32;
  uint64_t o = p.occ;
  for (int k = 0; ok && k < c; ++k) {
    const int s = pop_lsb(o), pc = piece_nibble(wlo, whi, k), pt = pc & 7;
    ok &= pt >= PAWN && pt <= KING;
    if (pc == make_piece(WHITE, KING)) ok &= wk < 0, wk = s;
    if (pc == make_piece(BLACK, KING)) ok &= bk < 0, bk = s;
  }
  if (!ok || wk < 0 || bk < 0) return 0;
  o = p.occ;
  for (int k = 0; k < c; ++k) {
    const int s = pop_lsb(o), pc = piece_nibble(wlo, whi, k);
    if (rows_white) rows_white[k] = (uint16_t)feature_index(WHITE, s, pc, wk);
    if (rows_black) rows_black[k] = (uint16_t)feature_index(BLACK, s, pc, bk);
  }
  return c;
}

GN_HD int wdl_material(const Board &B, const gn_eval_params &P) {
  int m = 0;
#pragma unroll
  for (int pt = PAWN; pt <= QUEEN; ++pt) m += P.wdl_piece_weight[pt - 1] * popcnt(B.byType[pt]);
  return m;
}
GN_HD int32_t wdl_to_cp(int32_t v, int material, const gn_eval_params &P) {
#pragma clang fp contract(off)
  const int lo = P.wdl_material_min, hi = P.wdl_material_max;
  const int mc = material < lo ? lo : material > hi ? hi : material;
  const double m = (double)mc / (double)P.wdl_material_anchor;
  const double a = ((P.wdl_a[0] * m + P.wdl_a[1]) * m + P.wdl_a[2]) * m + P.wdl_a[3];
  const double cp = round((double)(100 * (int64_t)v) / a);
  if (!(cp == cp)) return 0;
  return cp > 2147483647.0 ? 2147483647 : cp < -2147483647.0 ? -2147483647 : (int32_t)cp;
}

constexpr int32_t VALUE_MATE = 32000, VALUE_MATE_IN_MAX_PLY = 32000 - 246;
// ... 35 lines not shown
```

fishnet_amd/csrc/stream.hip:

```cpp
#include <stdio.h>
#include <stdlib.h>
#include <string.h>

#include <type_traits>

#include "device_util.h"
#include "kernels.h"

#ifndef GN_PLAN_WPE
#define GN_PLAN_WPE 4
#endif
#ifndef GN_SLICE_WPE
#define GN_SLICE_WPE 4
#endif
#define GN_PART_N GN_PART_SLICES
#ifndef GN_WCACHE
#define GN_WCACHE 1
#endif
#ifndef GN_EXPAND_WPE
#define GN_EXPAND_WPE (GN_RING == 4 ? 5 : 4)
#endif
#define GN_STR2(x) #x
#define GN_STR(x) GN_STR2(x)

#ifdef GN_STREAM_PROF
__device__ unsigned long long gn_sp[8];
#define SP_T() __builtin_amdgcn_s_memtime()
#define SP_ADD(k, v) atomicAdd(&gn_sp[k], (unsigned long long)(v))
#else
#define SP_T() 0ull
#define SP_ADD(k, v) (void)(v)
#endif
#ifdef GN_PLAN_PROF
__device__ unsigned long long gn_pp[4];
#define PP_T() __builtin_amdgcn_s_memtime()
#define PP_ADD(k, v) atomicAdd(&gn_pp[k], (unsigned long long)(v))
#else
#define PP_T() 0ull
#define PP_ADD(k, v) (void)(v)
#endif
#ifdef GN_XCD_PROF
__device__ unsigned long long gn_xp[32] = {0, 0, 0, 0, 0, 0, 0, 0, ~0ull, ~0ull, ~0ull, ~0ull, ~0ull, ~0ull, ~0ull, ~0ull};
#endif

#ifdef GN_FAULT_PLAN_BLOCK
__device__ int gn_fault_armed = 1;
#endif

namespace gn {
namespace ps {
constexpr uint32_t H_LAST = 1u << 18, H_X = 1u << 19,
                   H_PAR_E = H_X | 1u << 20, H_KST = H_X | 1u << 21, H_LDS_SH = 22;
constexpr uint32_t L_SCR = 1u << 31;
constexpr uint32_t M_ADD = 1u, M_SUB = 0xFFFFu;
constexpr uint32_t HZ = 1u << 16, HP = 2u << 16, HB = 3u << 16;
__device__ __forceinline__ uint32_t hs(int slot, int side, uint32_t xu, uint32_t hu) {
  return ((uint32_t)slot * xu + (uint32_t)side * hu) << H_LDS_SH;
}
constexpr bool lds_field16(int XS, int LC) {
  return XS % 16 == 0 && (LC / 2) % 16 == 0 && 15 * (XS / 16) + LC / 32 < 1024;
}
#ifndef GN_SLICE_XPAD
#define GN_SLICE_XPAD 0
#endif
constexpr int tile_xs(int L1, int SL) { return L1 / SL + 16 + (SL > 1 ? GN_SLICE_XPAD : 0); }
constexpr uint32_t field_xu(int L1, int SL) {
  return lds_field16(tile_xs(L1, SL), L1 / SL) ? (uint32_t)tile_xs(L1, SL) / 16 : 2u;
}
constexpr uint32_t field_hu(int L1, int SL) { return lds_field16(tile_xs(L1, SL), L1 / SL) ? (uint32_t)(L1 / SL) / 32 : 1u; }
__device__ __forceinline__ void wave_sync() {
  __builtin_amdgcn_fence(__ATOMIC_RELEASE, "wavefront");
  __builtin_amdgcn_wave_barrier();
  __builtin_amdgcn_fence(__ATOMIC_ACQUIRE, "wavefront");
}
}

constexpr int PLAN_WAVES = GN_FRONT_WG / 64;
template <int L1>
__global__ void __launch_bounds__(GN_FRONT_WG) __attribute__((amdgpu_waves_per_eu(GN_PLAN_WPE)))
    plan_kernel(NetDevice net, const gn_board *__restrict__ parents, const uint64_t *__restrict__ offsets,
                const ChildDelta *__restrict__ deltas, const uint8_t *__restrict__ need_parent,
                const uint8_t *__restrict__ need_child, const uint8_t *__restrict__ next_slot, uint32_t np, uint32_t K,
                uint32_t b0, uint32_t b1, int kc, const uint64_t *__restrict__ eoff, uint64_t *__restrict__ ent, TileDesc *__restrict__ tiles,
                uint32_t *__restrict__ btiles, unsigned long long *__restrict__ rows_out,
                unsigned long long *__restrict__ pads_out, uint32_t *__restrict__ err, int2 *__restrict__ pinfo,
                uint32_t xu, uint32_t hu) {
  using namespace ps;
  __shared__ uint32_t ksnap[PLAN_WAVES][128][8];
  __shared__ uint16_t prow_s[PLAN_WAVES][2][32];
  __shared__ uint32_t jrow_s[PLAN_WAVES][4][64];
  const int lane = threadIdx.x & 63, w = __builtin_amdgcn_readfirstlane((int)(threadIdx.x >> 6));
  const uint32_t blk = b0 + blockIdx.x * PLAN_WAVES + (uint32_t)w;
  if (blk >= b1) return;
  const __amdgpu_buffer_rsrc_t pst = __builtin_amdgcn_make_buffer_rsrc(
      (void *)net.psqt, 0, (int)((size_t)PSQT_BUCKETS * FT_ROWS * 4), 0x00020000);
  auto psqt = [&](uint32_t row, int bucket) -> int32_t {
#ifdef GN_AB_PLAN_NOPSQT
    return (int32_t)(row + bucket);
#endif
    return (int32_t)__builtin_amdgcn_raw_buffer_load_b32(pst, (bucket * (uint32_t)FT_ROWS + row) * 4, 0, 0);
  };
  const uint32_t pbeg = blk * K, pend = pbeg + K < np ? pbeg + K : np;
  const uint64_t us_b = pbeg + offsets[pbeg];
  const uint64_t rbeg = eoff[pbeg] + (uint64_t)ENT_SPARE * blk, rend = eoff[pend] + (uint64_t)ENT_SPARE * (blk + 1);
  uint2 *E = reinterpret_cast<uint2 *>(ent + rbeg);
  const uint32_t rtot = (uint32_t)(rend - rbeg);
  uint32_t bad = 0;
  TileDesc *T = tiles + us_b / 16 + (uint64_t)(K + 2) * blk;
  uint32_t safe0 = 0, safe1 = 0;
  constexpr uint32_t RS = ft_row_stride(L1);
  constexpr uint32_t LO_BIAS = (uint32_t)FT_BIAS_ROW * RS, LO_ZERO = (uint32_t)ZERO_ROW * RS;
  auto lo_scr = [](uint32_t r) -> uint32_t { return ((uint32_t)FT_ROWS + r) * RS | L_SCR; };
  const uint32_t rlast = rtot - 1;
  auto put = [&](int g, uint32_t i, uint32_t lo, uint32_t hi) {
    if ((lo & L_SCR) && i < (g ? safe1 : safe0)) bad |= 4u;
    const uint32_t ic = i < rlast ? i : rlast;
    const uint32_t x = g ? rlast - ic : ic;
    *reinterpret_cast<uint2 *>(reinterpret_cast<char *>(E) + (x << 3)) = make_uint2(lo, hi);
  };
  uint32_t ks0 = 0, ks1 = 0;
  auto kstate_of = [&](int hh, int ksq) -> int { return __builtin_amdgcn_readlane((int)(hh ? ks1 : ks0), ksq); };
  auto kstate_set = [&](int hh, int ksq, int v) {
    if (hh) ks1 = lane == ksq ? (uint32_t)v : ks1;
    else ks0 = lane == ksq ? (uint32_t)v : ks0;
  };
  uint16_t(*prow)[32] = prow_s[w];
  uint32_t len0 = 0, len1 = 0, tile_k = 0, p_first = pbeg, u_fill = 0, t_first = 0, tile_bm = 0;
  unsigned long long pp_a = 0, pp_b = 0, pp_c = 0, pp_d = 0;
  int t_fill = 0, carried = 0;
  uint32_t rows = 0, pads = 0, fpads = 0;
  auto pad_to = [&](int g, uint32_t target) {
    uint32_t &len = g ? len1 : len0;
    if (len < target) {
      pads += target - len;
      if ((uint32_t)lane < target - len) put(g, len + lane, LO_BIAS, 0u);
      len = target;
    }
  };

  char *const Tb = reinterpret_cast<char *>(T);
  auto tf = [&](uint32_t k, uint32_t field) -> char * { return Tb + (k * (uint32_t)sizeof(TileDesc) + field); };
  auto flush = [&]() {
    if (lane >= t_fill && lane < 16) *tf(tile_k, offsetof(TileDesc, meta) + lane) = 0;
    if (lane == 0) *reinterpret_cast<uint4 *>(tf(tile_k, 0)) = make_uint4(len0, len1, p_first, t_first);
    ++tile_k, t_fill = 0, tile_bm = 0;
  };

  struct In {
    uint32_t bd, a, b, c, d, m, nd;
  };
  auto word = [](const uint8_t *b) { return *reinterpret_cast<const uint32_t *>((uintptr_t)b & ~(uintptr_t)3); };
  auto byte_of = [](uint32_t wv, const uint8_t *b) { return (wv >> (8 * ((uintptr_t)b & 3))) & 0xFFu; };
  auto fetch = [&](uint32_t p) -> In {
    const uint64_t off = offsets[p];
    const uint32_t nch = (uint32_t)(offsets[p + 1] - off);
    const uint8_t *any = reinterpret_cast<const uint8_t *>(parents + p);
    In x = {0, 0, 0, 0, 0, 0, 0};
    if (lane < 7) x.bd = reinterpret_cast<const uint32_t *>(parents + p)[lane];
    if (lane == 0) {
      x.m = word(next_slot ? next_slot + p : any);
      x.nd = word(need_parent ? need_parent + p : any);
    } else if ((uint32_t)lane - 1 < nch) {
      const uint32_t *src = reinterpret_cast<const uint32_t *>(deltas + off + lane - 1);
      x.a = src[0], x.b = src[1], x.c = src[2], x.d = src[3], x.m = src[4];
      x.nd = word(need_child ? need_child + off + lane - 1 : any);
    }
    return x;
  };
  In xd = {0, 0, 0, 0, 0, 0, 0};
  if (pbeg < pend) xd = fetch(pbeg);
  for (uint32_t p = pbeg; p < pend; ++p) {
    unsigned long long pp_t = PP_T();
    const uint64_t off = offsets[p];
    const int nch = (int)(offsets[p + 1] - off), total = 1 + nch;
    gn_board pb = {};
    {
      uint32_t pw[7];
#pragma unroll
      for (int i = 0; i < 7; ++i) pw[i] = (uint32_t)__builtin_amdgcn_readlane((int)xd.bd, i);
      pb.occ = (uint64_t)pw[0] | (uint64_t)pw[1] << 32;
      __builtin_memcpy(pb.pc, &pw[2], 16);
      pb.stm_ep = (uint8_t)pw[6];
    }
    const uint32_t f0 =
        (need_parent ? byte_of((uint32_t)__builtin_amdgcn_readlane((int)xd.nd, 0), need_parent + p) : 1u) |
        (next_slot ? byte_of((uint32_t)__builtin_amdgcn_readlane((int)xd.m, 0), next_slot + p) : 255u) << 8;
    const bool pre = total <= 64;
    const int P = wave_features(pb, prow[0], prow[1], lane);
    ps::wave_sync();
    int want = 0;
    if (pre) want = lane == 0 ? (int)(f0 & 0xFF) : lane < total ? (int)(need_child ? byte_of(xd.nd, need_child + off + lane - 1) : 1u) : 0;
// ... 339 lines not shown
        int ne;
        if (hit) {
          const int nd = popcnt(bs) + popcnt(ba);
          ne = nd + 2;
          const int ps = 1 + popcnt(bs & lt), pa = 1 + popcnt(bs) + popcnt(ba & lt);
          if (lane == 0) put(g, base, lo_scr(kr), M_ADD | HZ | tw);
          if ((bs >> lane) & 1) put(g, base + ps, (uint32_t)feature_index(hh, lane, spc, kt) * RS, M_SUB | tw);
          if ((ba >> lane) & 1) put(g, base + pa, (uint32_t)row * RS, M_ADD | tw);
          if (lane == 0) put(g, base + ne - 1, LO_ZERO, kr | tw | H_KST | L);
          rows += (uint32_t)(nd + 1);
        } else {
          ne = cn + 1 + (kuse ? 1 : 0);
          if (lane == 0) put(g, base, LO_BIAS, M_ADD | HZ | tw);
          if (row >= 0 && pos < cn) put(g, base + 1 + pos, (uint32_t)row * RS, M_ADD | tw | (!kuse && pos == cn - 1 ? L : 0u));
          if (kuse && lane == 0) put(g, base + ne - 1, LO_ZERO, kr | tw | H_KST | L);
          rows += (uint32_t)(cn + 1);
        }
        if (kuse) {
          uint32_t x = (uint32_t)cpc << (4 * (lane & 7));
          x = or8(x);
          if ((lane & 7) == 0) ksnap[w][kci][lane >> 3] = x;
          kstate_set(hh, kt, 1 | g << 1);
          ps::wave_sync();
        }
        if (kuse) {
          uint32_t &sf = g ? safe1 : safe0;
          sf = base + (uint32_t)ne - 1 + GN_SCR_GAP;
        }
        if (g) len1 += (uint32_t)ne;
        else len0 += (uint32_t)ne;
      }
      while (jc < ntp - 1) close_tile(jc), ++jc, open_tile(jc);
      pp_d += PP_T() - pp_t, pp_t = PP_T();
      {
        const uint32_t rel = exc - (uint32_t)__shfl((int)exc, tile_lane0(tix));
        const uint32_t at0 = (uint32_t)__shfl((int)ts0, tix) + (rel & 0xFFFF);
        const uint32_t at1 = (uint32_t)__shfl((int)ts1, tix) + (rel >> 16);
        const uint32_t t0w = hs(t, cst != 0, xu, hu), t1w = hs(t, cst != 1, xu, hu);
        if (in && live) {
          auto delta = [&](int g, uint32_t at, uint32_t lo2, uint32_t hi2, int s, int n, bool hit, uint32_t tw,
                           uint32_t L) {
            const uint32_t i0 = lo2 & 0xFFFF, i1 = lo2 >> 16, i2 = hi2 & 0xFFFF, i3 = hi2 >> 16;
            auto cl = [](uint32_t r) { return (r < (uint32_t)FT_INPUTS ? r : (uint32_t)FT_BIAS_ROW) * RS; };
            const uint32_t r1 = cl(s >= 2 ? i1 : i2), r2 = cl(s >= 2 ? i2 : i3), r3 = cl(i3);
            const uint32_t f1 = s >= 2 ? M_SUB : M_ADD;
            if (!hit) {
              put(g, at, cl(i0), M_SUB | HP | tw | (n == 1 ? L : 0u));
              if (n > 1) put(g, at + 1, r1, f1 | tw | (n == 2 ? L : 0u));
              if (n > 2) put(g, at + 2, r2, M_ADD | tw | (n == 3 ? L : 0u));
              if (n > 3) put(g, at + 3, r3, M_ADD | tw | L);
            } else {
              put(g, at, r1, f1 | HB | tw | (n == 2 ? L : 0u));
              if (n > 2) put(g, at + 1, r2, M_ADD | tw | (n == 3 ? L : 0u));
              if (n > 3) put(g, at + 2, r3, M_ADD | tw | L);
            }
          };
          if ((kinds & 3) == 1) delta(0, at0, w0, w1, s0, n0, hit0, t0w, H_LAST | (nx ? H_PAR_E : 0u));
          if ((kinds >> 2) == 1) delta(1, at1, w2, w3, s1, n1, hit1, t1w, H_LAST | (nx ? H_PAR_E : 0u));
        }
      }
      uint32_t lbm = 0;
#pragma unroll
      for (int b = 0; b < 8; ++b)
        if (__ballot(tix == ntp - 1 && ((mybit >> b) & 1))) lbm |= 1u << b;
      if (ntp > 1) p_first = p, t_first = u_fill + (uint32_t)tile_lane0(ntp - 1);
      tile_k = tk0 + (uint32_t)(ntp - 1);
      t_fill = ntp == 1 ? tf0 + n_in : n_in - tile_lane0(ntp - 1);
      tile_bm = ntp == 1 ? tile_bm | lbm : lbm;
      u_fill += (uint32_t)n_in;
      pp_c += PP_T() - pp_t;
      if (t_fill == 16) flush();
    }
  }
  if (t_fill) flush();
#ifdef GN_FAULT_PLAN_BLOCK
  if (blk == (uint32_t)(GN_FAULT_PLAN_BLOCK) && tile_k > 0) {
    int armed = lane == 0 ? atomicExch(&gn_fault_armed, 0) : 0;
    if (__builtin_amdgcn_readfirstlane(armed)) {
      if (lane == 0) *reinterpret_cast<uint2 *>(tf(tile_k - 1, 0)) = make_uint2(rtot + 4096u, rtot + 4096u);
      bad |= 1u;
    }
  }
#endif
  if (lane == 0) btiles[blk] = tile_k;
  const uint32_t werr = __ballot(bad & 1u) ? 1u : 0u, werr4 = __ballot(bad & 4u) ? 4u : 0u;
  if (lane == 0) {
    if ((uint64_t)len0 + len1 > (uint64_t)(rtot - ENT_SPARE) || werr) atomicOr(err, 1u);
    if (werr4) atomicOr(err, 4u);
    if (rows_out) atomicAdd(rows_out, (unsigned long long)rows);
    if (pads_out && pads) atomicAdd(pads_out, (unsigned long long)pads);
    PP_ADD(0, pp_a), PP_ADD(1, pp_b), PP_ADD(2, pp_c), PP_ADD(3, pp_d);
    SP_ADD(6, pads), SP_ADD(7, fpads);
  }
  (void)pads, (void)fpads;
}

template <int L1, int SL = 1>
__global__ void __launch_bounds__(L1 / SL / 8) __attribute__((amdgpu_waves_per_eu(SL > 1 ? GN_SLICE_WPE : GN_EXPAND_WPE)))
    stream_eval_kernel(NetDevice net, const uint64_t *__restrict__ offsets, uint32_t np, uint32_t K, uint32_t b0,
                       uint32_t b1, int swz,
                       const uint64_t *__restrict__ eoff, const uint64_t *__restrict__ ent,
                       const TileDesc *__restrict__ tiles, const uint32_t *__restrict__ btiles,
                       const uint32_t *__restrict__ order, int2 *__restrict__ out_parent, int2 *__restrict__ out_child,
                       uint32_t *__restrict__ pool, int use_scr, uint32_t *__restrict__ err,
                       uint32_t *__restrict__ claim, int slice, int32_t *__restrict__ part, uint64_t npos,
                       int2 *__restrict__ pinfo) {
  using namespace ps;
  constexpr int LC = L1 / SL;
  constexpr int G = LC / 16;
  constexpr int NT = 2 * G, NW = NT / 64, TILE = 16, XS = tile_xs(L1, SL), KS = LC / 64,
                KPW = KS / NW;
  constexpr int KSF = L1 / 64;
  constexpr uint32_t RS = ft_row_stride(L1);
  static_assert(G % 64 == 0 && KS % NW == 0 && KPW % 2 == 0 && L1 % SL == 0, "geometry");
  const uint32_t cofs = SL > 1 ? (uint32_t)slice * (uint32_t)LC : 0u;
  __shared__ __attribute__((aligned(16))) uint8_t xt[TILE * XS];
  constexpr int AS = 20;
  __shared__ __attribute__((aligned(16))) int32_t acc0[2][16 * AS];
  __shared__ __attribute__((aligned(16))) uint8_t in1[2][TILE][32];
  __shared__ int32_t fwd[2][TILE];
  __shared__ uint32_t sslot, sblk;
  const int tid = threadIdx.x;
  const int wave = __builtin_amdgcn_readfirstlane(tid >> 6);
  const int hu = __builtin_amdgcn_readfirstlane((tid / G) & 1);
  for (int i = tid; i < 2 * 16 * AS; i += NT) (&acc0[0][0])[i] = 0;
  const uint32_t nblk = b1 - b0;
  const uint32_t vgrid = swz == 1 ? 8 * ((nblk + 7) / 8) : nblk;
  uint32_t v = blockIdx.x;
  if (swz == 0) {
    if (tid == 0) sblk = atomicAdd(claim, 1u);
    __syncthreads();
    v = sblk;
  } else if (swz == 2) {
    if (tid == 0) {
      uint32_t x;
      asm volatile("s_getreg_b32 %0, hwreg(HW_REG_XCC_ID)" : "=s"(x));
      x &= 7;
      const uint32_t per = (nblk + 7) / 8;
      uint32_t got = ~0u;
      for (uint32_t t = 0; t < 8 && got == ~0u; ++t) {
        const uint32_t y = (x + t) & 7, lo = y * per, hi = lo + per < nblk ? lo + per : nblk;
        if (lo >= hi || __hip_atomic_load(claim + y, __ATOMIC_RELAXED, __HIP_MEMORY_SCOPE_AGENT) >= hi - lo) continue;
        const uint32_t i = atomicAdd(claim + y, 1u);
        if (i < hi - lo) got = lo + i;
      }
      sblk = got;
    }
    __syncthreads();
    v = sblk;
  }
  if (v >= vgrid) return;
  uint32_t blk = v;
  if (swz == 1) {
    const uint32_t b8 = (nblk + 7) / 8;
    blk = (v & 7) * b8 + (v >> 3);
    if (blk >= nblk) return;
  }
  blk = order ? order[b0 + blk] : blk + b0;
  const uint32_t pbeg = blk * K, pend = pbeg + K < np ? pbeg + K : np;
  const uint64_t us_b = pbeg + offsets[pbeg];
  const uint32_t ntiles = btiles[blk];
  const TileDesc *T = tiles + us_b / 16 + (uint64_t)(K + 2) * blk;
  const uint64_t rbeg = eoff[pbeg] + (uint64_t)ENT_SPARE * blk, rend = eoff[pend] + (uint64_t)ENT_SPARE * (blk + 1);
  const uint32_t elim = (uint32_t)(rend - rbeg) - ENT_SPARE;
#ifdef GN_XCD_PROF
  const unsigned long long xp_t0 = __builtin_amdgcn_s_memrealtime();
#endif
  uint32_t scr = 0, my_slot = 0;
  if (use_scr) {
    if (tid == 0) {
      uint32_t x;
      asm volatile("s_getreg_b32 %0, hwreg(HW_REG_XCC_ID)" : "=s"(x));
      x &= 7;
      uint32_t *wd = pool + 8 * x;
      int got = -1;
      for (int it = 0; it < 4096 && got < 0; ++it) {
        const int wi = (int)((it + (v >> 3)) & 7);
        uint32_t cur = __hip_atomic_load(wd + wi, __ATOMIC_RELAXED, __HIP_MEMORY_SCOPE_AGENT);
        while (cur != 0xFFFFFFFFu) {
          const int bit = __builtin_ctz(~cur);
          const uint32_t old = __hip_atomic_fetch_or(wd + wi, 1u << bit, __ATOMIC_RELAXED, __HIP_MEMORY_SCOPE_AGENT);
          if (!(old & (1u << bit))) {
            got = (int)(x * POOL_PER_XCD + 32 * wi + bit);
            break;
          }
          cur = old | (1u << bit);
        }
        if (got < 0 && wi == 7) __builtin_amdgcn_s_sleep(4);
      }
      if (got < 0) atomicOr(err, 2u), got = 0;
      sslot = (uint32_t)got;
    }
    __syncthreads();
    my_slot = sslot;
    scr = (uint32_t)FT_ROWS + (uint32_t)SCR_ROWS * my_slot;
  }

  auto run_group = [&](auto hu_c) {
  constexpr int HU = decltype(hu_c)::value;
  uint32_t PA[8] = {0, 0, 0, 0, 0, 0, 0, 0}, BA[8] = {0, 0, 0, 0, 0, 0, 0, 0};
  constexpr int RD = SL > 1 ? GN_SLICE_RING : GN_RING;
  static_assert(RD == 4 || RD == 5 || RD == 6 || RD == 8, "ring depth");
  constexpr int RWAIT = 2 * (RD - 1), RWAIT_PV = 2 * RD;
  constexpr int GV = RD;
  ushort8 rlo[RD], rhi[RD];
  uint32_t eh[RD];
  uint32_t bq = 0;
  int4v wc[8];
  int cb = 8;
  const __amdgpu_buffer_rsrc_t w0r = __builtin_amdgcn_make_buffer_rsrc(
      (void *)net.w0f, 0, (int)((size_t)PSQT_BUCKETS * KSF * 1024), 0x00020000);
  const uint32_t wl16 = (uint32_t)(threadIdx.x & 63) * 16;
  auto wc_load = [&](int b) {
    const uint32_t so = ((uint32_t)b * KSF + (uint32_t)(24 * HU + 8 * slice)) * 1024u;
    asm volatile("buffer_load_dwordx4 %0, %8, %9, %10 offen\n\t"
                 "buffer_load_dwordx4 %1, %8, %9, %10 offen offset:1024\n\t"
                 "buffer_load_dwordx4 %2, %8, %9, %10 offen offset:2048\n\t"
                 "buffer_load_dwordx4 %3, %8, %9, %10 offen offset:3072\n\t"
                 "buffer_load_dwordx4 %4, %8, %9, %11 offen\n\t"
                 "buffer_load_dwordx4 %5, %8, %9, %11 offen offset:1024\n\t"
                 "buffer_load_dwordx4 %6, %8, %9, %11 offen offset:2048\n\t"
                 "buffer_load_dwordx4 %7, %8, %9, %11 offen offset:3072"
                 : "+v"(wc[0]), "+v"(wc[1]), "+v"(wc[2]), "+v"(wc[3]), "+v"(wc[4]), "+v"(wc[5]), "+v"(wc[6]),
                   "+v"(wc[7])
                 : "v"(wl16), "s"(w0r), "s"(so), "s"(so + 4096u));
  };
#define GN_WC_WAIT(N) asm volatile("s_waitcnt vmcnt(%8)" : "+v"(wc[0]), "+v"(wc[1]), "+v"(wc[2]), "+v"(wc[3]), \
                                   "+v"(wc[4]), "+v"(wc[5]), "+v"(wc[6]), "+v"(wc[7]) : "n"(N))
  typedef uint32_t u8e __attribute__((ext_vector_type(2 * GV), aligned(8)));
  typedef const __attribute__((address_space(4))) u8e cu8e;
  typedef const __attribute__((address_space(4))) uint64_t cu64;
  cu64 *EL = (cu64 *)(HU ? ent + rend : ent + rbeg);
  auto group = [&](uint32_t i) -> u8e { return *(cu8e *)(HU ? EL - GV - i : EL + i); };
  auto elo = [&](const u8e v, int r) -> uint32_t { return HU ? v[2 * (GV - 1 - r)] : v[2 * r]; };
  auto ehi = [&](const u8e v, int r) -> uint32_t { return HU ? v[2 * (GV - 1 - r) + 1] : v[2 * r + 1]; };
  int tl0 = tid;
  asm volatile("" : "+v"(tl0));
  const int jt = tl0 % G;
  const uint32_t j16 = 16 * jt + cofs;
  typedef int sq4 __attribute__((ext_vector_type(4)));
  const uint64_t ftp = (uint64_t)(uintptr_t)net.ft;
  const sq4 rsq = {__builtin_amdgcn_readfirstlane((int)(uint32_t)ftp),
                   __builtin_amdgcn_readfirstlane((int)(uint32_t)(ftp >> 32) & 0xFFFF),
                   (int)(((size_t)ZERO_ROW + 1) * RS), 0x00020000};
  const uint32_t scr_off = (scr - (uint32_t)FT_ROWS) * RS - L_SCR;
  auto offset = [&](uint32_t lo, uint32_t h) -> uint32_t {
    (void)h;
// ... 411 lines not shown
          l2[i] = w2l * l + w2h * hh;
        }
#pragma unroll
        for (int off = 8; off; off >>= 1)
#pragma unroll
          for (int i = 0; i < 4; ++i) l2[i] = wadd(l2[i], __shfl_xor(l2[i], off, 16));
        if (row == 0) {
#pragma unroll
          for (int i = 0; i < 4; ++i) {
            const int pos = 4 * kg + i;
            const uint32_t m = (mw[pos >> 2] >> (8 * (pos & 3))) & 0xFF;
            if ((m & 1) && (int)((m >> 1) & 7) == b) {
              const int32_t positional = wadd(wadd(b2v, l2[i]), fwd[buf][pos]);
              const int32_t psqt = (int32_t)((uint32_t)pq[i].x - (uint32_t)pq[i].y) / 2;
              const int2 val = make_int2(psqt / 16, positional / 16);
              const uint32_t P = p_first + (uint32_t)__builtin_popcount(pm & ((2u << pos) - 1)) - (pm & 1);
              if ((pm >> pos) & 1) out_parent[P] = val;
              else out_child[u0 + pos - P - 1 + adj[i]] = val;
            }
          }
        }
      }
      ++bq;
    }
    sp_l += SP_T() - t2;
  }
#ifdef GN_STREAM_PROF
  if ((tid & 63) == 0) {
    SP_ADD(0, sp_s), SP_ADD(1, sp_w), SP_ADD(2, sp_l);
    if (wave == 0) SP_ADD(3, ntiles), SP_ADD(4, sp_m), SP_ADD(5, sp_n);
  }
#else
  (void)sp_s, (void)sp_w, (void)sp_l, (void)sp_m, (void)sp_n, (void)sp_e0, (void)sp_e1;
#endif
  };
  if (hu) run_group(std::integral_constant<int, 1>{});
  else run_group(std::integral_constant<int, 0>{});
  if (use_scr) {
    asm volatile("s_waitcnt vmcnt(0)" ::: "memory");
    __syncthreads();
    if (tid == 0)
      __hip_atomic_fetch_and(pool + 8 * (my_slot / POOL_PER_XCD) + (my_slot % POOL_PER_XCD) / 32,
                             ~(1u << (my_slot % 32)), __ATOMIC_RELAXED, __HIP_MEMORY_SCOPE_AGENT);
  }
#ifdef GN_XCD_PROF
  if (tid == 0) {
    uint32_t x;
    asm volatile("s_getreg_b32 %0, hwreg(HW_REG_XCC_ID)" : "=s"(x));
    x &= 7;
    const unsigned long long t1 = __builtin_amdgcn_s_memrealtime();
    atomicMax(&gn_xp[x], t1);
    atomicMin(&gn_xp[8 + x], xp_t0);
    atomicAdd(&gn_xp[16 + x], ntiles ? (unsigned long long)T[ntiles - 1].e_end[0] + T[ntiles - 1].e_end[1] : 0ull);
    atomicAdd(&gn_xp[24 + x], 1ull);
  }
#endif
}

template <int SL>
__global__ void __launch_bounds__(256) slice_finish_kernel(NetDevice net, const int32_t *__restrict__ part,
                                                           const int2 *__restrict__ pinfo, uint64_t npos, uint32_t np,
                                                           int2 *__restrict__ out_parent, int2 *__restrict__ out_child) {
  __shared__ int4v w1s[8 * 32 * 2];
  stage_fc1(w1s, net);
  __syncthreads();
  const uint64_t q = (uint64_t)blockIdx.x * blockDim.x + threadIdx.x;
  if (q >= npos) return;
  const int2 info = pinfo[q];
  if (info.y < 0) return;
  const int2 val = slice_finish_one<GN_PART_N>(net, w1s, part, npos, q, info);
  if (q < np) out_parent[q] = val;
  else out_child[q - np] = val;
}

hipError_t launch_plan_stream(const NetDevice &net, const PlanStreamArgs &a, int phases, hipStream_t s) {
  const size_t n = a.n;
  if (!n) return hipSuccess;
  const bool do_plan = phases & PLAN_PHASE, do_stream = phases & STREAM_PHASE;
  if (n >= 0x80000000ull) return hipErrorInvalidValue;
  const uint32_t K = a.chain_k > 1 && a.next_slot ? (uint32_t)a.chain_k : 1u;
  const uint8_t *next_slot = K > 1 ? a.next_slot : nullptr;
  const int kc = K > 1 ? a.kc : 0;
  const int scr = K > 1 && a.kc;
  const uint32_t nb = (uint32_t)((n + K - 1) / K), B0 = 0, B1 = nb;
  const unsigned pg = (nb + PLAN_WAVES - 1) / PLAN_WAVES, g = a.swz == 1 ? 8 * ((nb + 7) / 8) : nb + nb / 16 + 8;
  auto stream_done = [&] {
    if (a.fin) (void)hipEventRecord(a.fin, s);
    if (a.streamed) (void)hipEventRecord(a.streamed, s);
  };
  if (net.L1 == 3072) {
    const bool sliced = a.slices == 3 && a.part && a.pinfo;
    if (do_plan) {
      if (sliced) {
        hipError_t e = hipMemsetAsync(a.pinfo, 0xFF, a.npos * sizeof(int2), s);
        if (e != hipSuccess) return e;
      }
      hipLaunchKernelGGL((plan_kernel<3072>), dim3(pg), dim3(GN_FRONT_WG), 0, s, net, a.parents, a.offsets, a.deltas,
                         a.need_parent, a.need_child, next_slot, (uint32_t)n, K, B0, B1, kc, a.eoff, a.ent, a.tiles,
                         a.btiles, a.rows_out, a.pads_out, a.err, sliced ? a.pinfo : nullptr,
                         sliced ? ps::field_xu(3072, 3) : ps::field_xu(3072, 1), sliced ? ps::field_hu(3072, 3) : ps::field_hu(3072, 1));
      if (a.mid) (void)hipEventRecord(a.mid, s);
    }
    if (!do_stream) {
    } else if (sliced) {
      for (int sl = 0; sl < 3; ++sl)
        hipLaunchKernelGGL((stream_eval_kernel<3072, 3>), dim3(g), dim3(128), 0, s, net, a.offsets, (uint32_t)n, K, B0,
                           B1, a.swz, a.eoff, a.ent, a.tiles, a.btiles, a.order, a.out_parent, a.out_child, a.pool, scr,
                           a.err, a.pool + 64 + 8 * sl, sl, a.part, (uint64_t)a.npos, a.pinfo);
      stream_done();
      if (a.finish)
        hipLaunchKernelGGL((slice_finish_kernel<3>), dim3((unsigned)((a.npos + 255) / 256)), dim3(256), 0, s, net,
                           a.part, a.pinfo, (uint64_t)a.npos, (uint32_t)n, a.out_parent, a.out_child);
    } else {
      hipLaunchKernelGGL((stream_eval_kernel<3072>), dim3(g), dim3(384), 0, s, net, a.offsets, (uint32_t)n, K, B0, B1,
                         a.swz, a.eoff, a.ent, a.tiles, a.btiles, a.order, a.out_parent, a.out_child, a.pool, scr, a.err,
                         a.pool + 64, 0, nullptr, (uint64_t)0, nullptr);
      stream_done();
    }
  } else if (net.L1 == 1024) {
    if (do_plan) {
      hipLaunchKernelGGL((plan_kernel<1024>), dim3(pg), dim3(GN_FRONT_WG), 0, s, net, a.parents, a.offsets, a.deltas,
                         a.need_parent, a.need_child, next_slot, (uint32_t)n, K, B0, B1, kc, a.eoff, a.ent, a.tiles,
                         a.btiles, a.rows_out, a.pads_out, a.err, nullptr, ps::field_xu(1024, 1), ps::field_hu(1024, 1));
      if (a.mid) (void)hipEventRecord(a.mid, s);
    }
    if (do_stream) {
      hipLaunchKernelGGL((stream_eval_kernel<1024>), dim3(g), dim3(128), 0, s, net, a.offsets, (uint32_t)n, K, B0, B1,
                         a.swz, a.eoff, a.ent, a.tiles, a.btiles, a.order, a.out_parent, a.out_child, a.pool, scr, a.err,
                         a.pool + 64, 0, nullptr, (uint64_t)0, nullptr);
      stream_done();
    }
  } else {
    return hipErrorInvalidValue;
  }
#ifdef GN_PLAN_PROF
  {
    unsigned long long c[4];
    (void)hipStreamSynchronize(s);
    (void)hipMemcpyFromSymbol(c, HIP_SYMBOL(gn_pp), sizeof(c));
    fprintf(stderr, "plan prof: wave-cycles setup %llu slots %llu delta puts %llu king jobs %llu\n", c[0], c[1],
            c[2], c[3]);
    memset(c, 0, sizeof(c));
    (void)hipMemcpyToSymbol(HIP_SYMBOL(gn_pp), c, sizeof(c));
  }
#endif
#ifdef GN_XCD_PROF
  {
    unsigned long long c[32];
    (void)hipStreamSynchronize(s);
    (void)hipMemcpyFromSymbol(c, HIP_SYMBOL(gn_xp), sizeof(c));
    unsigned long long t0 = ~0ull;
    for (int x = 0; x < 8; ++x) t0 = c[8 + x] < t0 ? c[8 + x] : t0;
    fprintf(stderr, "xcd prof:");
    for (int x = 0; x < 8; ++x)
      fprintf(stderr, " [%d] end %.2f ms start %.2f ms entries %llu wgs %llu;", x, (c[x] - t0) * 1e-5,
              (c[8 + x] - t0) * 1e-5, c[16 + x], c[24 + x]);
    fprintf(stderr, "\n");
    for (int x = 0; x < 8; ++x) c[x] = 0, c[8 + x] = ~0ull, c[16 + x] = 0, c[24 + x] = 0;
    (void)hipMemcpyToSymbol(HIP_SYMBOL(gn_xp), c, sizeof(c));
  }
#endif
#ifdef GN_STREAM_PROF
  {
    unsigned long long c[8];
    (void)hipStreamSynchronize(s);
    (void)hipMemcpyFromSymbol(c, HIP_SYMBOL(gn_sp), sizeof(c));
    fprintf(stderr, "stream prof: wave-cycles stream %llu barrier %llu ls %llu; tiles %llu; "
                    "entries max-list %llu sum %llu (balance %.3f), no-op entries %llu scratch-order + %llu tile-end\n",
            c[0], c[1], c[2], c[3], c[4], c[5], c[5] ? 2.0 * c[4] / c[5] : 0.0, c[6], c[7]);
    memset(c, 0, sizeof(c));
    (void)hipMemcpyToSymbol(HIP_SYMBOL(gn_sp), c, sizeof(c));
  }
#endif
  return hipGetLastError();
}

}
```

fishnet_amd/gpu_nnue.py:

```python
from __future__ import annotations

import ctypes as C
import os

import numpy as np

HERE = os.path.dirname(os.path.abspath(__file__))
LIB_PATH = os.environ.get("GPU_NNUE_LIB", os.path.join(HERE, "lib", "libgpu_nnue.so"))

MODE_FULL, MODE_BIG, MODE_SMALL = 0, 1, 2
FLAG_IN_CHECK, FLAG_SMALLNET, FLAG_BAD_FEN, FLAG_REEVAL, FLAG_SKIPPED = 1, 2, 4, 8, 16
FLAG_MATE, FLAG_NO_SCORE, FLAG_SEARCHED, FLAG_NO_MOVES = 32, 64, 128, 256
ERRORS = {-1: "INVALID", -2: "IO", -3: "FORMAT", -4: "HIP", -5: "NOMEM", -6: "CAPACITY",
          -7: "NODEVICE", -8: "NONET", -9: "ILLEGAL_MOVE"}
E_INVALID, E_IO, E_FORMAT, E_HIP, E_NOMEM, E_CAPACITY, E_NODEVICE, E_NONET, E_ILLEGAL_MOVE = -1, -2, -3, -4, -5, -6, -7, -8, -9

EVAL_DTYPE = np.dtype([("psqt", "<i4"), ("positional", "<i4"), ("final_v", "<i4"), ("final_cp", "<i4"),
                       ("score", "<i4"), ("flags", "<u2"), ("best_move", "<u2")])
BOARD_DTYPE = np.dtype([("occ", "<u8"), ("pc", "u1", (16,)), ("stm_ep", "u1"), ("reserved", "u1"),
                        ("castle", "<u2"), ("rule50", "<u2"), ("fullmove", "<u2")])
CHILD_DTYPE = np.dtype([("psqt", "<i4"), ("positional", "<i4"), ("cp_flags", "<i4")])
CHILD_VIEW_DTYPE = np.dtype([("psqt", "<i4"), ("positional", "<i4"), ("final_cp", "<i4"), ("flags", "<u2")])
EVAL_SIZE, BOARD_SIZE, CHILD_SIZE = EVAL_DTYPE.itemsize, BOARD_DTYPE.itemsize, CHILD_DTYPE.itemsize
assert EVAL_SIZE == 24 and BOARD_SIZE == 32 and CHILD_SIZE == 12
ABI_VERSION = 4

EXPORTS = ["gn_load_net", "gn_load_net_memory", "gn_free", "gn_last_error", "gn_abi_version",
           "gn_get_eval_params", "gn_set_eval_params", "gn_net_info", "gn_evaluate_batch",
           "gn_evaluate_batch_mode", "gn_expand_and_evaluate", "gn_perft", "gn_pack_fens",
           "gn_board_to_fen", "gn_random_positions", "gn_evaluate_device", "gn_expand_device",
           "gn_device_alloc", "gn_device_free", "gn_memcpy_h2d", "gn_memcpy_d2h", "gn_synchronize",
           "gn_time_evaluate_device", "gn_random_positions_device", "gn_set_option", "gn_get_option",
           "gn_time_expand_device", "gn_random_games_device", "gn_replay_game", "gn_evaluate_games",
           "gn_net_sha256", "gn_partition", "gn_checksum_device",
           "gn_boards_to_fens", "gn_load_net_archive", "gn_archive_read", "gn_expand2_device",
           "gn_random_games_uci"]
OPT_INCREMENTAL_CHILDREN, OPT_XCD_SWIZZLE, OPT_KING_SORT, OPT_CHAIN, OPT_KING_CACHE = 1, 2, 3, 4, 5
OPT_CHUNK_PARENTS, OPT_COALESCE, OPT_STREAM_SLICES, OPT_FAST_BATCH, OPT_EXPAND_PIPELINE = 6, 7, 8, 9, 10
STAT_PLAN_NS, STAT_STREAM_NS, STAT_SCRATCH_PADS, STAT_FINISH_NS = 101, 102, 103, 104
STAT_BATCH_LAUNCHES, STAT_BATCH_CALLS, STAT_FAST_BATCHES, STAT_FAST_FALLBACKS = 117, 118, 119, 120
HOST_STAGES = {"parse": 110, "upload": 111, "replay": 112, "compute": 113, "download": 114, "tail": 115, "total": 116}
EXPAND_STAGES = ["count_scan", "total_readback", "write_children", "classify", "small_net", "big_net", "finalize",
                 "score"]


def decode_children(raw) -> np.ndarray:
    raw = np.asarray(raw, dtype=CHILD_DTYPE)
    out = np.empty(raw.shape, dtype=CHILD_VIEW_DTYPE)
    cf = raw["cp_flags"].astype(np.int64)
    out["psqt"], out["positional"] = raw["psqt"], raw["positional"]
    out["final_cp"] = ((cf & 0xFFFFFF) ^ 0x800000) - 0x800000
    out["flags"] = (cf >> 24) & 0xFF
    return out


def children_from_evals(ev) -> np.ndarray:
    ev = np.asarray(ev, dtype=EVAL_DTYPE)
    out = np.empty(ev.shape, dtype=CHILD_VIEW_DTYPE)
    out["psqt"], out["positional"], out["final_cp"] = ev["psqt"], ev["positional"], ev["final_cp"]
    out["flags"] = ev["flags"] & 0xFF
    return out


class GnError(RuntimeError):
    def __init__(self, code, msg):
        super().__init__(f"gpu_nnue error {code} ({ERRORS.get(code, '?')}): {msg}")
        self.code = code


class EvalParams(C.Structure):
    _fields_ = [(n, C.c_int32) for n in (
        "small_net_threshold", "psqt_weight", "positional_weight", "reeval_threshold",
        "complexity_div_small", "complexity_div_big", "material_pawn_small", "material_pawn_big",
        "material_base", "rule50_div", "value_clamp")] + [
        ("piece_value", C.c_int32 * 5), ("wdl_a", C.c_double * 4), ("wdl_material_min", C.c_int32),
        ("wdl_material_max", C.c_int32), ("wdl_material_anchor", C.c_int32), ("wdl_piece_weight", C.c_int32 * 5)]


class GnGame(C.Structure):
    _fields_ = [("root_fen", C.c_char_p), ("uci_moves", C.c_char_p),
                ("skip_positions", C.POINTER(C.c_uint32)), ("n_skip", C.c_size_t)]


def _games_array(games):
    keep, arr = [], (GnGame * max(len(games), 1))()
    for i, g in enumerate(games):
        root, moves, skip = (tuple(g) + ((),) * 3)[:3]
        mv = moves if isinstance(moves, str) else " ".join(moves or ())
        sk = (C.c_uint32 * max(len(skip), 1))(*skip)
        keep += [root.encode(), mv.encode(), sk]
        arr[i].root_fen, arr[i].uci_moves = keep[-3], keep[-2]
        arr[i].skip_positions = C.cast(sk, C.POINTER(C.c_uint32))
        arr[i].n_skip = len(skip)
    return arr, keep


_lib = None


def lib():
    global _lib
    if _lib is not None:
        return _lib
    if not os.path.exists(LIB_PATH):
        raise ImportError(f"libgpu_nnue.so not built at {LIB_PATH}: run `python -m fishnet_amd.build`")
    L = C.CDLL(LIB_PATH)
    vp, sz, i32 = C.c_void_p, C.c_size_t, C.c_int
    sig = {
        "gn_load_net": [C.c_char_p, C.c_char_p, vp, i32, C.POINTER(vp)],
        "gn_load_net_memory": [vp, sz, vp, sz, vp, i32, C.POINTER(vp)],
        "gn_free": [vp],
        "gn_last_error": [],
        "gn_abi_version": [],
        "gn_get_eval_params": [vp, C.POINTER(EvalParams)],
        "gn_set_eval_params": [vp, C.POINTER(EvalParams)],
        "gn_net_info": [vp, C.POINTER(i32), C.POINTER(C.c_uint32), C.POINTER(i32), C.POINTER(C.c_uint32)],
        "gn_evaluate_batch": [vp, vp, sz, vp],
        "gn_evaluate_batch_mode": [vp, vp, sz, i32, vp],
        "gn_expand_and_evaluate": [vp, vp, sz, i32, vp, vp, vp, vp, sz],
        "gn_perft": [vp, C.c_char_p, i32, C.POINTER(C.c_uint64)],
        "gn_pack_fens": [vp, sz, vp, vp],
        "gn_board_to_fen": [vp, C.c_char_p, sz],
# ... 386 lines not shown
```

include/gpu_nnue.h:

```cpp
#ifndef GPU_NNUE_H
#define GPU_NNUE_H
#include <stddef.h>
#include <stdint.h>

#ifdef __cplusplus
extern "C" {
#endif

#define GN_ABI_VERSION 4

#if defined(__GNUC__)
#define GN_API __attribute__((visibility("default")))
#else
#define GN_API
#endif

#define GN_OK 0
#define GN_E_INVALID (-1)
#define GN_E_IO (-2)
#define GN_E_FORMAT (-3)
#define GN_E_HIP (-4)
#define GN_E_NOMEM (-5)
#define GN_E_CAPACITY (-6)
#define GN_E_NODEVICE (-7)
#define GN_E_NONET (-8)
#define GN_E_ILLEGAL_MOVE (-9)

#define GN_MODE_FULL 0
#define GN_MODE_BIG 1
#define GN_MODE_SMALL 2

#define GN_OPT_CHUNK_PARENTS 6
#define GN_OPT_COALESCE 7
#define GN_OPT_FAST_BATCH 9
#define GN_OPT_EXPAND_PIPELINE 10
#define GN_OPT_INCREMENTAL_CHILDREN 1
#define GN_OPT_XCD_SWIZZLE 2
#define GN_OPT_KING_SORT 3
#define GN_OPT_KING_CACHE 5
#define GN_OPT_CHAIN 4
#define GN_OPT_STREAM_SLICES 8

#define GN_STAT_PLAN_NS 101
#define GN_STAT_STREAM_NS 102
#define GN_STAT_FINISH_NS 104
#define GN_STAT_SCRATCH_PADS 103
#define GN_STAT_HOST_PARSE_NS 110
#define GN_STAT_HOST_UPLOAD_NS 111
#define GN_STAT_HOST_REPLAY_NS 112
#define GN_STAT_HOST_COMPUTE_NS 113
#define GN_STAT_HOST_DOWNLOAD_NS 114
#define GN_STAT_HOST_TAIL_NS 115
#define GN_STAT_HOST_TOTAL_NS 116
#define GN_STAT_BATCH_LAUNCHES 117
#define GN_STAT_BATCH_CALLS 118
#define GN_STAT_FAST_BATCHES 119
#define GN_STAT_FAST_FALLBACKS 120

#define GN_FLAG_IN_CHECK 1u
#define GN_FLAG_SMALLNET 2u
#define GN_FLAG_BAD_FEN 4u
#define GN_FLAG_REEVAL 8u
#define GN_FLAG_SKIPPED 16u
#define GN_FLAG_MATE 32u
#define GN_FLAG_NO_SCORE 64u
#define GN_FLAG_SEARCHED 128u
#define GN_FLAG_NO_MOVES 256u

typedef struct gn_eval {
  int32_t psqt;
  int32_t positional;
  int32_t final_v;
  int32_t final_cp;
  int32_t score;
  uint16_t flags;
  uint16_t best_move;
} gn_eval;

typedef struct gn_child {
  int32_t psqt;
  int32_t positional;
  int32_t cp_flags;
} gn_child;
#define GN_CHILD_FINAL_CP(c) ((int32_t)((uint32_t)(c).cp_flags << 8) >> 8)
#define GN_CHILD_FLAGS(c) ((uint32_t)(c).cp_flags >> 24)

typedef struct gn_board {
  uint64_t occ;
  uint8_t pc[16];
  uint8_t stm_ep;
  uint8_t reserved;
  uint16_t castle;
  uint16_t rule50;
  uint16_t fullmove;
} gn_board;

typedef struct gn_eval_params {
  int32_t small_net_threshold;
  int32_t psqt_weight;
  int32_t positional_weight;
  int32_t reeval_threshold;
  int32_t complexity_div_small;
  int32_t complexity_div_big;
  int32_t material_pawn_small;
  int32_t material_pawn_big;
  int32_t material_base;
  int32_t rule50_div;
  int32_t value_clamp;
  int32_t piece_value[5];
  double wdl_a[4];
  int32_t wdl_material_min;
  int32_t wdl_material_max;
  int32_t wdl_material_anchor;
  int32_t wdl_piece_weight[5];
} gn_eval_params;

typedef struct gn_ctx gn_ctx;

GN_API int gn_load_net(const char *big_path, const char *small_path, const int *devices, int n_devices,
                gn_ctx **out);
GN_API int gn_load_net_memory(const uint8_t *big, size_t big_len, const uint8_t *small, size_t small_len,
                       const int *devices, int n_devices, gn_ctx **out);
GN_API int gn_load_net_archive(const char *archive_path, const char *big_member, const char *small_member,
                               const int *devices, int n_devices, gn_ctx **out);
GN_API int gn_archive_read(const char *archive_path, const char *member, uint8_t *buf, size_t cap, size_t *size);
GN_API void gn_free(gn_ctx *ctx);
GN_API const char *gn_last_error(void);
GN_API int gn_abi_version(void);
// ... 71 lines not shown
```

rust/gpu-nnue-sys/src/lib.rs:

```rust
#![allow(non_camel_case_types)]
use std::os::raw::{c_char, c_int, c_void};

pub const GN_ABI_VERSION: c_int = 4;

pub const GN_OK: c_int = 0;
pub const GN_E_INVALID: c_int = -1;
pub const GN_E_IO: c_int = -2;
pub const GN_E_FORMAT: c_int = -3;
pub const GN_E_HIP: c_int = -4;
pub const GN_E_NOMEM: c_int = -5;
pub const GN_E_CAPACITY: c_int = -6;
pub const GN_E_NODEVICE: c_int = -7;
pub const GN_E_NONET: c_int = -8;
pub const GN_E_ILLEGAL_MOVE: c_int = -9;

pub const GN_MODE_FULL: c_int = 0;
pub const GN_MODE_BIG: c_int = 1;
pub const GN_MODE_SMALL: c_int = 2;

pub const GN_OPT_INCREMENTAL_CHILDREN: c_int = 1;
pub const GN_OPT_XCD_SWIZZLE: c_int = 2;
pub const GN_OPT_KING_SORT: c_int = 3;
pub const GN_OPT_CHAIN: c_int = 4;
pub const GN_OPT_KING_CACHE: c_int = 5;
pub const GN_OPT_CHUNK_PARENTS: c_int = 6;
pub const GN_OPT_COALESCE: c_int = 7;
pub const GN_OPT_STREAM_SLICES: c_int = 8;
pub const GN_OPT_FAST_BATCH: c_int = 9;
pub const GN_OPT_EXPAND_PIPELINE: c_int = 10;
pub const GN_STAT_PLAN_NS: c_int = 101;
pub const GN_STAT_STREAM_NS: c_int = 102;
pub const GN_STAT_SCRATCH_PADS: c_int = 103;
pub const GN_STAT_FINISH_NS: c_int = 104;
pub const GN_STAT_HOST_PARSE_NS: c_int = 110;
pub const GN_STAT_HOST_UPLOAD_NS: c_int = 111;
pub const GN_STAT_HOST_REPLAY_NS: c_int = 112;
pub const GN_STAT_HOST_COMPUTE_NS: c_int = 113;
pub const GN_STAT_HOST_DOWNLOAD_NS: c_int = 114;
pub const GN_STAT_HOST_TAIL_NS: c_int = 115;
pub const GN_STAT_HOST_TOTAL_NS: c_int = 116;
pub const GN_STAT_BATCH_LAUNCHES: c_int = 117;
pub const GN_STAT_BATCH_CALLS: c_int = 118;
pub const GN_STAT_FAST_BATCHES: c_int = 119;
pub const GN_STAT_FAST_FALLBACKS: c_int = 120;

pub const GN_FLAG_IN_CHECK: u16 = 1;
pub const GN_FLAG_SMALLNET: u16 = 2;
pub const GN_FLAG_BAD_FEN: u16 = 4;
pub const GN_FLAG_REEVAL: u16 = 8;
pub const GN_FLAG_SKIPPED: u16 = 16;
pub const GN_FLAG_MATE: u16 = 32;
pub const GN_FLAG_NO_SCORE: u16 = 64;
pub const GN_FLAG_SEARCHED: u16 = 128;
pub const GN_FLAG_NO_MOVES: u16 = 256;

#[repr(C)]
#[derive(Clone, Copy, Default, Debug, PartialEq, Eq)]
pub struct gn_eval {
    pub psqt: i32,
    pub positional: i32,
    pub final_v: i32,
    pub final_cp: i32,
    pub score: i32,
    pub flags: u16,
    pub best_move: u16,
}

#[repr(C)]
#[derive(Clone, Copy, Default, Debug, PartialEq, Eq)]
pub struct gn_child {
    pub psqt: i32,
    pub positional: i32,
    pub cp_flags: i32,
}

impl gn_child {
    pub fn final_cp(&self) -> i32 {
        ((self.cp_flags as u32) << 8) as i32 >> 8
    }
    pub fn flags(&self) -> u16 {
        ((self.cp_flags as u32) >> 24) as u16
    }
}

#[repr(C)]
#[derive(Clone, Copy, Default, Debug, PartialEq, Eq)]
pub struct gn_board {
    pub occ: u64,
    pub pc: [u8; 16],
    pub stm_ep: u8,
    pub reserved: u8,
    pub castle: u16,
    pub rule50: u16,
    pub fullmove: u16,
}

#[repr(C)]
#[derive(Clone, Copy, Default, Debug, PartialEq)]
pub struct gn_eval_params {
    pub small_net_threshold: i32,
    pub psqt_weight: i32,
    pub positional_weight: i32,
    pub reeval_threshold: i32,
    pub complexity_div_small: i32,
    pub complexity_div_big: i32,
    pub material_pawn_small: i32,
    pub material_pawn_big: i32,
    pub material_base: i32,
    pub rule50_div: i32,
    pub value_clamp: i32,
    pub piece_value: [i32; 5],
    pub wdl_a: [f64; 4],
    pub wdl_material_min: i32,
    pub wdl_material_max: i32,
    pub wdl_material_anchor: i32,
    pub wdl_piece_weight: [i32; 5],
// ... 105 lines not shown
```

Before: 855.2 million.

## Replace fixed-K parent chains with variable-length blocks cut at king-bucket changes

Replaces the fixed chain length K with a device-built block table (flags, scan, scatter to block-first indices), which all plan, stream and child-write kernels now use. An optional cut mode starts a new block whenever the parent's king-bucket pair changes, so incremental accumulator chains avoid refreshes across bucket boundaries. Block metadata is packed into per-block uint4 records, and the XCD partition can follow bucket-sorted boundaries. Cut mode is off by default, so the default path gets the table overhead (an extra scan and readback) but no new block boundaries.

```diff
diff --git a/fishnet_amd/csrc/gpu_nnue.hip b/fishnet_amd/csrc/gpu_nnue.hip
--- a/fishnet_amd/csrc/gpu_nnue.hip
+++ b/fishnet_amd/csrc/gpu_nnue.hip
@@ -222,6 +222,8 @@
   EvalBufs eb;
   DevBuf<gn_board> children;
   int chain_k = 1;
+  uint32_t nblk = 0;
+  bool cut = false;
   int slices = 1;
   bool planned = false;
   uint64_t etot = 0;
@@ -233,9 +235,11 @@
   DevBuf<uint64_t> ent, eoff;
   DevBuf<TileDesc> tiles;
   DevBuf<uint32_t> btiles, border;
+  DevBuf<uint32_t> bfirst, xb;
   void release() {
     perr.release(), pstat.release();
     ent.release(), eoff.release(), tiles.release(), btiles.release(), border.release();
+    bfirst.release(), xb.release();
     counts.release(), offsets.release(), owner.release(), unpacked.release(), moves_tmp.release();
     pinfo.release(), p_osm.release(), p_obg.release(), p_nsm.release(), p_nbg.release(), eb.release();
     children.release();
@@ -270,6 +274,7 @@
   DevBuf<uint32_t> pool;
   DevBuf<uint16_t> bkeys, bkeys2;
   DevBuf<uint32_t> bidx;
+  DevBuf<uint32_t> bflag, bpos;
   hipEvent_t done = nullptr;
   hipStream_t done_on = nullptr;
   float plan_ms = 0, stream_ms = 0, finish_ms = 0;
@@ -343,6 +348,9 @@
 #define GN_MAX_LEADERS 1
 #endif
 constexpr int MAX_LEADERS = GN_MAX_LEADERS;
+#ifndef GN_BLOCK_CUT_DEFAULT
+#define GN_BLOCK_CUT_DEFAULT 0
+#endif
 struct BatchReq {
   const gn_board *boards;
   size_t n;
@@ -374,6 +382,7 @@
   int king_sort = 1;
   int chain = 81;
   bool king_cache = true;
+  bool block_cut = GN_BLOCK_CUT_DEFAULT != 0;
   int stream_slices = 3;
   int64_t chunk_parents = 0;
   int l1[2] = {0, 0};
@@ -475,7 +484,7 @@
     d.kkeys.release(), d.kkeys2.release(), d.kidx.release(), d.kperm.release();
     d.nslot.release();
     d.ebound.release(), d.pool.release();
-    d.bkeys.release(), d.bkeys2.release(), d.bidx.release();
+    d.bkeys.release(), d.bkeys2.release(), d.bidx.release(), d.bflag.release(), d.bpos.release();
     d.lv[0].release(), d.lv[1].release();
     for (auto &row : d.fast)
       for (auto &pair : row)
@@ -703,6 +712,7 @@
   unsigned long long *rows = nullptr;
   bool deltas = false;
   int chain_k = 1;
+  bool cut = false;
   bool plan = false;
   bool skip_internal = false;
   size_t limit = SIZE_MAX;
@@ -728,9 +738,19 @@
   HIP_TRY(launch_count_children(parents, n, d.tables, x.counts.p, s, x.planned ? d.ebound.p : nullptr));
   HIP_TRY(exclusive_scan_u64(x.counts.p, x.offsets.p, n + 1, x.scan_tmp, x.scan_bytes, s));
   if (x.planned) HIP_TRY(exclusive_scan_u64(d.ebound.p, x.eoff.p, n + 1, x.scan_tmp, x.scan_bytes, s));
+  const bool table = x.planned || x.chain_k > 1;
+  x.nblk = 0, x.cut = x.planned && o.cut;
+  if (table) {
+    HIP_TRY(d.bflag.ensure(n + 1));
+    HIP_TRY(d.bpos.ensure(n + 1));
+    HIP_TRY(x.bfirst.ensure(n + 1));
+    HIP_TRY(block_table(parents, n, (uint32_t)x.chain_k, x.cut, d.bflag.p, d.bpos.p, x.bfirst.p,
+                        x.scan_tmp, x.scan_bytes, s));
+  }
   if (o.ev) HIP_TRY(hipEventRecord(o.ev[0], s));
   uint64_t t = 0;
   HIP_TRY(hipMemcpyAsync(&t, x.offsets.p + n, sizeof(t), hipMemcpyDeviceToHost, s));
+  if (table) HIP_TRY(hipMemcpyAsync(&x.nblk, d.bpos.p + n, sizeof(uint32_t), hipMemcpyDeviceToHost, s));
   if (x.planned) HIP_TRY(hipMemcpyAsync(&x.etot, x.eoff.p + n, sizeof(uint64_t), hipMemcpyDeviceToHost, s));
   HIP_TRY(hipStreamSynchronize(s));
   *total = (size_t)t;
@@ -752,8 +772,8 @@
   x.child_moves = moves;
   if (t) {
     HIP_TRY(launch_write_children(parents, n, d.tables, x.offsets.p, 0, t, children, moves, x.owner.p,
-                                  o.deltas ? d.deltas.p : nullptr, x.chain_k > 1 ? d.nslot.p : nullptr, x.chain_k,
-                                  o.rows, s, x.unpacked.p));
+                                  o.deltas ? d.deltas.p : nullptr, x.chain_k > 1 ? d.nslot.p : nullptr,
+                                  x.chain_k > 1 ? d.bflag.p : nullptr, o.rows, s, x.unpacked.p));
   }
   if (o.ev) HIP_TRY(hipEventRecord(o.ev[2], s));
   return GN_OK;
@@ -762,7 +782,7 @@
 static GenOpts gen_opts(const gn_ctx *ctx, Dev &d, size_t n, int mode, size_t limit) {
   GenOpts g;
   g.deltas = ctx->incremental, g.chain_k = chain_len(ctx, d, n), g.plan = plan_path(ctx, d, mode);
-  g.skip_internal = mode == GN_MODE_BIG, g.limit = limit;
+  g.cut = ctx->block_cut, g.skip_internal = mode == GN_MODE_BIG, g.limit = limit;
   return g;
 }
 
@@ -798,7 +818,7 @@
   const uint64_t *off = x.offsets.p;
   const ChildDelta *dl = d.deltas.p;
   const bool f = mode == GN_MODE_FULL;
-  const size_t K = (size_t)std::max(1, x.chain_k), nblk = (n + K - 1) / K;
+  const size_t nblk = x.nblk;
   const bool ordered = ctx->king_sort && nblk > 1;
   auto plan_args = [&] {
     PlanStreamArgs a;
@@ -806,6 +826,7 @@
     a.need_parent = f ? x.p_nbg.p : nullptr, a.need_child = f ? x.eb.nbg.p : nullptr;
     a.out_parent = x.p_obg.p, a.out_child = x.eb.obg.p;
     a.next_slot = x.chain_k > 1 ? d.nslot.p : nullptr, a.chain_k = x.chain_k, a.kc = ctx->king_cache ? 1 : 0;
+    a.bfirst = x.bfirst.p, a.nblk = x.nblk;
     a.eoff = x.eoff.p, a.ent = x.ent.p, a.tiles = x.tiles.p, a.btiles = x.btiles.p;
     a.pool = d.pool.p, a.err = x.perr.p, a.rows_out = o.rows, a.pads_out = x.pstat.p;
     a.slices = x.slices, a.npos = n + total;
@@ -843,8 +864,8 @@
     x.slices = 1;
     if (mode != GN_MODE_SMALL && x.planned) {
       HIP_TRY(x.ent.ensure(x.etot + (size_t)ENT_SPARE * (nblk + 1)));
-      HIP_TRY(x.tiles.ensure((n + total) / 16 + (K + 2) * nblk + 2));
-      HIP_TRY(x.btiles.ensure(nblk + 1));
+      HIP_TRY(x.tiles.ensure((n + total) / 16 + n + 2 * nblk + 2));
+      HIP_TRY(x.btiles.ensure(8 * (nblk + 1)));
       HIP_TRY(d.pool.ensure(88));
       if (d.net[BIG].L1 == 3072 && ctx->stream_slices == 3) {
         const size_t need = (size_t)GN_PART_SLICES * 16 * (n + total);
@@ -862,8 +883,9 @@
         HIP_TRY(d.bkeys2.ensure(nblk));
         HIP_TRY(d.bidx.ensure(nblk));
         HIP_TRY(x.border.ensure(nblk));
-        HIP_TRY(block_order(parents, n, (uint32_t)K, (uint32_t)nblk, d.bkeys.p, d.bidx.p, d.bkeys2.p, x.border.p,
-                            x.sort_tmp, x.sort_bytes, s));
+        if (x.cut) HIP_TRY(x.xb.ensure(9));
+        HIP_TRY(block_order(parents, n, x.bfirst.p, (uint32_t)nblk, d.bkeys.p, d.bidx.p, d.bkeys2.p, x.border.p,
+                            d.bflag.p, d.bpos.p, x.cut ? x.xb.p : nullptr, x.sort_tmp, x.sort_bytes, s));
       }
       PlanStreamArgs a = plan_args();
       a.mid = ev ? ev[4] : nullptr;
@@ -881,7 +903,7 @@
       if (ev && (phases & EXP_FRONT) == 0) HIP_TRY(hipEventRecord(ev[7], s));
       PlanStreamArgs a = plan_args();
       a.swz = (ctx->swizzle >> 2) & 1 ? 1 : (ctx->swizzle >> 3) & 1 ? 2 : 0;
-      a.order = ordered ? x.border.p : nullptr;
+      a.order = ordered ? x.border.p : nullptr, a.xb = ordered && x.cut ? x.xb.p : nullptr;
       a.fin = ev ? ev[6] : nullptr, a.streamed = o.streamed, a.finish = !fused;
       HIP_TRY(launch_plan_stream(d.net[BIG], a, STREAM_PHASE, s));
     } else {
@@ -945,7 +967,7 @@
   HIP_TRY(L.ce.ensure(std::max<uint64_t>(t, 1)));
   HIP_TRY(L.sv.ensure(std::max<uint64_t>(t, 1)));
   HIP_TRY(launch_write_children(L.boards.p, m, d.tables, L.offsets.p, 0, t, L.children.p, L.moves.p, L.owner.p,
-                                nullptr, nullptr, 1, nullptr, s));
+                                nullptr, nullptr, nullptr, nullptr, s));
   int rc = evaluate_on(ctx, d, L.children.p, t, mode, L.ce.p, s, nullptr);
   if (rc) return rc;
   if ((rc = resolve_scores(ctx, d, L.children.p, t, mode, L.ce.p, L.sv.p, s, depth - 1)) != GN_OK) return rc;
@@ -2495,6 +2517,9 @@
   case GN_OPT_KING_CACHE:
     ctx->king_cache = value != 0;
     return GN_OK;
+  case GN_OPT_BLOCK_CUT:
+    ctx->block_cut = value != 0;
+    return GN_OK;
   case GN_OPT_CHAIN:
     if (value < -(1 << 20) || value > (1 << 20)) return fail(GN_E_INVALID, "chain length out of range");
     ctx->chain = (int)value;
@@ -2537,6 +2562,18 @@
   case GN_OPT_KING_CACHE:
     *value = ctx->king_cache;
     return GN_OK;
+  case GN_OPT_BLOCK_CUT:
+    *value = ctx->block_cut;
+    return GN_OK;
+  case GN_STAT_BLOCKS: {
+    int64_t sum = 0;
+    for (auto &dp : ctx->devs) {
+      std::lock_guard<std::mutex> lk(dp->mu);
+      sum += dp->cur.nblk;
+    }
+    *value = sum;
+    return GN_OK;
+  }
   case GN_OPT_CHAIN:
     *value = ctx->chain;
     return GN_OK;
diff --git a/fishnet_amd/csrc/kernels.h b/fishnet_amd/csrc/kernels.h
--- a/fishnet_amd/csrc/kernels.h
+++ b/fishnet_amd/csrc/kernels.h
@@ -34,8 +34,11 @@
                            unsigned long long *rows_out = nullptr, const gn_eval_params *cls = nullptr,
                            uint8_t *need_small = nullptr, uint8_t *need_big = nullptr);
 hipError_t launch_checksum(const void *p, size_t bytes, unsigned long long *out, hipStream_t s);
-hipError_t block_order(const gn_board *parents, size_t n, uint32_t K, uint32_t nblk, uint16_t *keys, uint32_t *idx,
-                       uint16_t *keys_out, uint32_t *order, void *&temp, size_t &temp_bytes, hipStream_t s);
+hipError_t block_table(const gn_board *parents, size_t n, uint32_t K, int cut, uint32_t *flags, uint32_t *pos,
+                       uint32_t *bfirst, void *&temp, size_t &temp_bytes, hipStream_t s);
+hipError_t block_order(const gn_board *parents, size_t n, const uint32_t *bfirst, uint32_t nblk, uint16_t *keys,
+                       uint32_t *idx, uint16_t *keys_out, uint32_t *order, uint32_t *len, uint32_t *spos, uint32_t *xb,
+                       void *&temp, size_t &temp_bytes, hipStream_t s);
 hipError_t king_sort(const gn_board *boards, size_t n, uint64_t *keys, uint32_t *idx, uint64_t *keys_out,
                      uint32_t *perm, bool placement, void *&temp, size_t &temp_bytes, hipStream_t s);
 hipError_t launch_expand_net(const NetDevice &net, const gn_board *parents, size_t n, const uint64_t *offsets,
@@ -60,6 +63,8 @@
   int2 *out_parent = nullptr, *out_child = nullptr;
   const uint8_t *next_slot = nullptr;
   int chain_k = 1;
+  const uint32_t *bfirst = nullptr;
+  uint32_t nblk = 0;
   int kc = 0;
   const uint64_t *eoff = nullptr;
   uint64_t *ent = nullptr;
@@ -70,6 +75,7 @@
   unsigned long long *rows_out = nullptr;
   unsigned long long *pads_out = nullptr;
   const uint32_t *order = nullptr;
+  const uint32_t *xb = nullptr;
   int slices = 1;
   int32_t *part = nullptr;
   size_t npos = 0;
@@ -117,8 +123,8 @@
                                  hipStream_t s, uint64_t *ebound = nullptr);
 hipError_t launch_write_children(const gn_board *boards, size_t n, const Tables *tables, const uint64_t *offsets,
                                  size_t c0, size_t nc, gn_board *children, uint16_t *moves, uint32_t *owner,
-                                 ChildDelta *deltas, uint8_t *next_slot, int chain_k, unsigned long long *rows,
-                                 hipStream_t s, Board *unpacked = nullptr);
+                                 ChildDelta *deltas, uint8_t *next_slot, const uint32_t *bflags,
+                                 unsigned long long *rows, hipStream_t s, Board *unpacked = nullptr);
 hipError_t launch_count_sum(const gn_board *boards, size_t n, const Tables *tables,
                             unsigned long long *total, hipStream_t s);
 hipError_t launch_random_positions(uint64_t seed, size_t first, size_t n, int max_plies, const Tables *tables,
diff --git a/fishnet_amd/csrc/kernels.hip b/fishnet_amd/csrc/kernels.hip
--- a/fishnet_amd/csrc/kernels.hip
+++ b/fishnet_amd/csrc/kernels.hip
@@ -1082,8 +1082,9 @@
 
 __global__ void child_moves_kernel(const gn_board *__restrict__ boards, size_t n, const Tables *__restrict__ tables,
                                    const uint64_t *__restrict__ offsets, uint16_t *__restrict__ moves,
-                                   uint32_t *__restrict__ owner, uint8_t *__restrict__ next_slot, int chain_k,
-                                   unsigned long long *__restrict__ rows, Board *__restrict__ unpacked) {
+                                   uint32_t *__restrict__ owner, uint8_t *__restrict__ next_slot,
+                                   const uint32_t *__restrict__ bflags, unsigned long long *__restrict__ rows,
+                                   Board *__restrict__ unpacked) {
   __shared__ Tables T;
   load_tables(T, tables);
   const size_t i = (size_t)blockIdx.x * blockDim.x + threadIdx.x;
@@ -1143,7 +1144,7 @@
   if (next_slot) next_slot[i] = (uint8_t)slot;
   if (rows) {
     unsigned long long r = 2ull * popcnt(occ);
-    if (slot != 255 && chain_k > 1 && (i + 1) % (size_t)chain_k != 0) r -= 2ull * popcnt(N.byType[0]) - 2;
+    if (slot != 255 && bflags && !bflags[i + 1]) r -= 2ull * popcnt(N.byType[0]) - 2;
     atomicAdd(rows, r);
   }
 }
@@ -1340,12 +1341,12 @@
 
 hipError_t launch_write_children(const gn_board *boards, size_t n, const Tables *tables, const uint64_t *offsets,
                                  size_t c0, size_t nc, gn_board *children, uint16_t *moves, uint32_t *owner,
-                                 ChildDelta *deltas, uint8_t *next_slot, int chain_k, unsigned long long *rows,
-                                 hipStream_t s, Board *unpacked) {
+                                 ChildDelta *deltas, uint8_t *next_slot, const uint32_t *bflags,
+                                 unsigned long long *rows, hipStream_t s, Board *unpacked) {
   if (!n) return hipSuccess;
   if (!moves || !owner) return hipErrorInvalidValue;
   hipLaunchKernelGGL(child_moves_kernel, dim3(blocks_for(n, GN_FRONT_WG)), dim3(GN_FRONT_WG), 0, s, boards, n, tables, offsets, moves,
-                     owner, next_slot, chain_k, rows, unpacked);
+                     owner, next_slot, bflags, rows, unpacked);
   if (nc)
     hipLaunchKernelGGL(child_boards_kernel, dim3(blocks_for(nc, GN_FRONT_WG)), dim3(GN_FRONT_WG), 0, s, boards, c0, nc, moves, owner,
                        children, deltas, rows, unpacked);
@@ -1424,12 +1425,28 @@
                      temp, temp_bytes, s);
 }
 
-__global__ void block_keys_kernel(const gn_board *__restrict__ parents, size_t n, uint32_t K, uint32_t nblk,
-                                  uint16_t *__restrict__ keys, uint32_t *__restrict__ idx) {
-  const uint32_t b = blockIdx.x * blockDim.x + threadIdx.x;
-  if (b >= nblk) return;
-  const size_t pb = (size_t)b * K, pe = pb + K < n ? pb + K : n;
-  const gn_board p = parents[pb + (pe - pb) / 2];
+template <class T>
+static hipError_t exclusive_scan_t(const T *counts, T *offsets, size_t n1, void *&temp, size_t &temp_bytes,
+                                   hipStream_t s) {
+  size_t need = 0;
+  hipError_t e = hipcub::DeviceScan::ExclusiveSum(nullptr, need, counts, offsets, n1, s);
+  if (e != hipSuccess) return e;
+  if (need > temp_bytes) {
+    if (temp) (void)hipFree(temp);
+    temp = nullptr;
+    temp_bytes = 0;
+    if ((e = hipMalloc(&temp, need)) != hipSuccess) return e;
+    temp_bytes = need;
+  }
+  return hipcub::DeviceScan::ExclusiveSum(temp, temp_bytes, counts, offsets, n1, s);
+}
+
+hipError_t exclusive_scan_u64(const uint64_t *counts, uint64_t *offsets, size_t n1, void *&temp, size_t &temp_bytes,
+                              hipStream_t s) {
+  return exclusive_scan_t(counts, offsets, n1, temp, temp_bytes, s);
+}
+
+__device__ __forceinline__ uint32_t bucket_pair(const gn_board &p) {
   uint64_t wlo, whi;
   piece_words(p, wlo, whi);
   uint64_t o = p.occ;
@@ -1440,18 +1457,85 @@
     if (pc == make_piece(WHITE, KING)) wk = sq;
     if (pc == make_piece(BLACK, KING)) bk = sq;
   }
-  keys[b] = (uint16_t)(wk << 6 | bk);
+  return (uint32_t)(king_bucket(WHITE, wk) << 5 | king_bucket(BLACK, bk));
+}
+
+#ifndef GN_CUT_MIN_LEN
+#define GN_CUT_MIN_LEN 1
+#endif
+__global__ void block_flags_kernel(const gn_board *__restrict__ parents, size_t n, uint32_t K, int cut,
+                                   uint32_t *__restrict__ flags) {
+  const size_t i = (size_t)blockIdx.x * blockDim.x + threadIdx.x;
+  if (i > n) return;
+  uint32_t f = 0;
+  if (i < n) {
+    f = i % K == 0;
+    if (!f && cut) {
+      const uint32_t key = bucket_pair(parents[i]);
+      f = key != bucket_pair(parents[i - 1]);
+      for (size_t j = i + 1; f && j < i + GN_CUT_MIN_LEN; ++j)
+        f = j < n && j % K != 0 && bucket_pair(parents[j]) == key;
+    }
+  }
+  flags[i] = f;
+}
+
+__global__ void block_scatter_kernel(const uint32_t *__restrict__ flags, const uint32_t *__restrict__ pos, size_t n,
+                                     uint32_t *__restrict__ bfirst) {
+  const size_t i = (size_t)blockIdx.x * blockDim.x + threadIdx.x;
+  if (i > n) return;
+  if (i == n || flags[i]) bfirst[pos[i]] = (uint32_t)i;
+}
+
+hipError_t block_table(const gn_board *parents, size_t n, uint32_t K, int cut, uint32_t *flags, uint32_t *pos,
+                       uint32_t *bfirst, void *&temp, size_t &temp_bytes, hipStream_t s) {
+  hipLaunchKernelGGL(block_flags_kernel, dim3(blocks_for(n + 1, 256)), dim3(256), 0, s, parents, n, K ? K : 1u, cut,
+                     flags);
+  hipError_t e = hipGetLastError();
+  if (e != hipSuccess) return e;
+  if ((e = exclusive_scan_t(flags, pos, n + 1, temp, temp_bytes, s)) != hipSuccess) return e;
+  hipLaunchKernelGGL(block_scatter_kernel, dim3(blocks_for(n + 1, 256)), dim3(256), 0, s, flags, pos, n, bfirst);
+  return hipGetLastError();
+}
+
+__global__ void block_keys_kernel(const gn_board *__restrict__ parents, const uint32_t *__restrict__ bfirst,
+                                  uint32_t nblk, uint16_t *__restrict__ keys, uint32_t *__restrict__ idx) {
+  const uint32_t b = blockIdx.x * blockDim.x + threadIdx.x;
+  if (b >= nblk) return;
+  const uint32_t pb = bfirst[b], pe = bfirst[b + 1];
+  keys[b] = (uint16_t)bucket_pair(parents[pb + (pe - pb) / 2]);
   idx[b] = b;
 }
 
-hipError_t block_order(const gn_board *parents, size_t n, uint32_t K, uint32_t nblk, uint16_t *keys, uint32_t *idx,
-                       uint16_t *keys_out, uint32_t *order, void *&temp, size_t &temp_bytes, hipStream_t s) {
+__global__ void block_len_kernel(const uint32_t *__restrict__ bfirst, const uint32_t *__restrict__ order,
+                                 uint32_t nblk, uint32_t *__restrict__ len) {
+  const uint32_t j = blockIdx.x * blockDim.x + threadIdx.x;
+  if (j > nblk) return;
+  len[j] = j < nblk ? bfirst[order[j] + 1] - bfirst[order[j]] : 0u;
+}
+
+__global__ void block_bounds_kernel(const uint32_t *__restrict__ spos, uint32_t nblk, uint32_t n,
+                                    uint32_t *__restrict__ xb) {
+  const uint32_t j = blockIdx.x * blockDim.x + threadIdx.x;
+  if (j > nblk) return;
+  if (j == 0) xb[0] = 0;
+  if (j == nblk) xb[8] = nblk;
+  for (uint32_t e = 1; e < 8; ++e) {
+    const uint32_t t = (uint32_t)((uint64_t)n * e / 8);
+    if (spos[j] >= t && (j == 0 || spos[j - 1] < t)) xb[e] = j;
+  }
+}
+
+hipError_t block_order(const gn_board *parents, size_t n, const uint32_t *bfirst, uint32_t nblk, uint16_t *keys,
+                       uint32_t *idx, uint16_t *keys_out, uint32_t *order, uint32_t *len, uint32_t *spos, uint32_t *xb,
+                       void *&temp, size_t &temp_bytes, hipStream_t s) {
   if (!nblk) return hipSuccess;
-  hipLaunchKernelGGL(block_keys_kernel, dim3(blocks_for(nblk, GN_FRONT_WG)), dim3(GN_FRONT_WG), 0, s, parents, n, K, nblk, keys, idx);
+  hipLaunchKernelGGL(block_keys_kernel, dim3(blocks_for(nblk, GN_FRONT_WG)), dim3(GN_FRONT_WG), 0, s, parents, bfirst,
+                     nblk, keys, idx);
   hipError_t e = hipGetLastError();
   if (e != hipSuccess) return e;
   size_t need = 0;
-  e = hipcub::DeviceRadixSort::SortPairs(nullptr, need, keys, keys_out, idx, order, (int)nblk, 0, 12, s);
+  e = hipcub::DeviceRadixSort::SortPairs(nullptr, need, keys, keys_out, idx, order, (int)nblk, 0, 10, s);
   if (e != hipSuccess) return e;
   if (need > temp_bytes) {
     if (temp) (void)hipFree(temp);
@@ -1460,22 +1544,13 @@
     if ((e = hipMalloc(&temp, need)) != hipSuccess) return e;
     temp_bytes = need;
   }
-  return hipcub::DeviceRadixSort::SortPairs(temp, temp_bytes, keys, keys_out, idx, order, (int)nblk, 0, 12, s);
-}
-
-hipError_t exclusive_scan_u64(const uint64_t *counts, uint64_t *offsets, size_t n1, void *&temp, size_t &temp_bytes,
-                              hipStream_t s) {
-  size_t need = 0;
-  hipError_t e = hipcub::DeviceScan::ExclusiveSum(nullptr, need, counts, offsets, n1, s);
-  if (e != hipSuccess) return e;
-  if (need > temp_bytes) {
-    if (temp) (void)hipFree(temp);
-    temp = nullptr;
-    temp_bytes = 0;
-    if ((e = hipMalloc(&temp, need)) != hipSuccess) return e;
-    temp_bytes = need;
-  }
-  return hipcub::DeviceScan::ExclusiveSum(temp, temp_bytes, counts, offsets, n1, s);
+  e = hipcub::DeviceRadixSort::SortPairs(temp, temp_bytes, keys, keys_out, idx, order, (int)nblk, 0, 10, s);
+  if (e != hipSuccess || !xb) return e;
+  hipLaunchKernelGGL(block_len_kernel, dim3(blocks_for(nblk + 1, 256)), dim3(256), 0, s, bfirst, order, nblk, len);
+  if ((e = hipGetLastError()) != hipSuccess) return e;
+  if ((e = exclusive_scan_t(len, spos, (size_t)nblk + 1, temp, temp_bytes, s)) != hipSuccess) return e;
+  hipLaunchKernelGGL(block_bounds_kernel, dim3(blocks_for(nblk + 1, 256)), dim3(256), 0, s, spos, nblk, (uint32_t)n, xb);
+  return hipGetLastError();
 }
 
 hipError_t launch_expand_net(const NetDevice &net, const gn_board *parents, size_t n, const uint64_t *offsets,
diff --git a/fishnet_amd/csrc/nnue.h b/fishnet_amd/csrc/nnue.h
--- a/fishnet_amd/csrc/nnue.h
+++ b/fishnet_amd/csrc/nnue.h
@@ -43,11 +43,15 @@
   const int8_t *w0f;
 };
 
+GN_HD int king_bucket(int persp, int ksq) {
+  const int kf = ksq & 7;
+  const int rel_rank = (ksq >> 3) ^ (persp ? 7 : 0);
+  return 4 * (7 - rel_rank) + (kf < 4 ? kf : 7 - kf);
+}
 GN_HD int feature_index(int persp, int sq, int pc, int ksq) {
   const int kf = ksq & 7;
   const int orient = (kf < 4 ? 7 : 0) ^ (persp ? 56 : 0);
-  const int rel_rank = (ksq >> 3) ^ (persp ? 7 : 0);
-  const int bucket = 4 * (7 - rel_rank) + (kf < 4 ? kf : 7 - kf);
+  const int bucket = king_bucket(persp, ksq);
   const int pt = pc & 7;
   const int plane = pt == KING ? 10 : 2 * (pt - 1) + ((pc >> 3) != persp);
   return (sq ^ orient) + 64 * plane + 704 * bucket;
diff --git a/fishnet_amd/csrc/stream.hip b/fishnet_amd/csrc/stream.hip
--- a/fishnet_amd/csrc/stream.hip
+++ b/fishnet_amd/csrc/stream.hip
@@ -80,8 +80,8 @@
 __global__ void __launch_bounds__(GN_FRONT_WG) __attribute__((amdgpu_waves_per_eu(GN_PLAN_WPE)))
     plan_kernel(NetDevice net, const gn_board *__restrict__ parents, const uint64_t *__restrict__ offsets,
                 const ChildDelta *__restrict__ deltas, const uint8_t *__restrict__ need_parent,
-                const uint8_t *__restrict__ need_child, const uint8_t *__restrict__ next_slot, uint32_t np, uint32_t K,
-                uint32_t b0, uint32_t b1, int kc, const uint64_t *__restrict__ eoff, uint64_t *__restrict__ ent, TileDesc *__restrict__ tiles,
+                const uint8_t *__restrict__ need_child, const uint8_t *__restrict__ next_slot,
+                const uint32_t *__restrict__ bfirst, uint32_t np, uint32_t K, uint32_t b0, uint32_t b1, int kc, const uint64_t *__restrict__ eoff, uint64_t *__restrict__ ent, TileDesc *__restrict__ tiles,
                 uint32_t *__restrict__ btiles, unsigned long long *__restrict__ rows_out,
                 unsigned long long *__restrict__ pads_out, uint32_t *__restrict__ err, int2 *__restrict__ pinfo,
                 uint32_t xu, uint32_t hu) {
@@ -100,13 +100,13 @@
 #endif
     return (int32_t)__builtin_amdgcn_raw_buffer_load_b32(pst, (bucket * (uint32_t)FT_ROWS + row) * 4, 0, 0);
   };
-  const uint32_t pbeg = blk * K, pend = pbeg + K < np ? pbeg + K : np;
+  const uint32_t pbeg = bfirst[blk], pend = bfirst[blk + 1];
   const uint64_t us_b = pbeg + offsets[pbeg];
   const uint64_t rbeg = eoff[pbeg] + (uint64_t)ENT_SPARE * blk, rend = eoff[pend] + (uint64_t)ENT_SPARE * (blk + 1);
   uint2 *E = reinterpret_cast<uint2 *>(ent + rbeg);
   const uint32_t rtot = (uint32_t)(rend - rbeg);
   uint32_t bad = 0;
-  TileDesc *T = tiles + us_b / 16 + (uint64_t)(K + 2) * blk;
+  TileDesc *T = tiles + us_b / 16 + pbeg + 2ull * blk;
   uint32_t safe0 = 0, safe1 = 0;
   constexpr uint32_t RS = ft_row_stride(L1);
   constexpr uint32_t LO_BIAS = (uint32_t)FT_BIAS_ROW * RS, LO_ZERO = (uint32_t)ZERO_ROW * RS;
@@ -612,7 +612,11 @@
     }
   }
 #endif
-  if (lane == 0) btiles[blk] = tile_k;
+  if (lane == 0) {
+    uint4 *bi = reinterpret_cast<uint4 *>(btiles) + 2 * (size_t)blk;
+    bi[0] = make_uint4(pbeg, tile_k, rtot - ENT_SPARE, 0u);
+    bi[1] = make_uint4((uint32_t)us_b, (uint32_t)(us_b >> 32), (uint32_t)rbeg, (uint32_t)(rbeg >> 32));
+  }
   const uint32_t werr = __ballot(bad & 1u) ? 1u : 0u, werr4 = __ballot(bad & 4u) ? 4u : 0u;
   if (lane == 0) {
     if ((uint64_t)len0 + len1 > (uint64_t)(rtot - ENT_SPARE) || werr) atomicOr(err, 1u);
@@ -627,8 +631,8 @@
 
 template <int L1, int SL = 1>
 __global__ void __launch_bounds__(L1 / SL / 8) __attribute__((amdgpu_waves_per_eu(SL > 1 ? GN_SLICE_WPE : GN_EXPAND_WPE)))
-    stream_eval_kernel(NetDevice net, const uint64_t *__restrict__ offsets, uint32_t np, uint32_t K, uint32_t b0,
-                       uint32_t b1, int swz,
+    stream_eval_kernel(NetDevice net, const uint64_t *__restrict__ offsets, const uint32_t *__restrict__ bfirst,
+                       const uint32_t *__restrict__ xb, uint32_t np, uint32_t b0, uint32_t b1, int swz,
                        const uint64_t *__restrict__ eoff, const uint64_t *__restrict__ ent,
                        const TileDesc *__restrict__ tiles, const uint32_t *__restrict__ btiles,
                        const uint32_t *__restrict__ order, int2 *__restrict__ out_parent, int2 *__restrict__ out_child,
@@ -669,7 +673,9 @@
       const uint32_t per = (nblk + 7) / 8;
       uint32_t got = ~0u;
       for (uint32_t t = 0; t < 8 && got == ~0u; ++t) {
-        const uint32_t y = (x + t) & 7, lo = y * per, hi = lo + per < nblk ? lo + per : nblk;
+        const uint32_t y = (x + t) & 7;
+        const uint32_t lo = xb ? (xb[y] < nblk ? xb[y] : nblk) : y * per;
+        const uint32_t hi = xb ? (xb[y + 1] < nblk ? xb[y + 1] : nblk) : lo + per < nblk ? lo + per : nblk;
         if (lo >= hi || __hip_atomic_load(claim + y, __ATOMIC_RELAXED, __HIP_MEMORY_SCOPE_AGENT) >= hi - lo) continue;
         const uint32_t i = atomicAdd(claim + y, 1u);
         if (i < hi - lo) got = lo + i;
@@ -687,12 +693,15 @@
     if (blk >= nblk) return;
   }
   blk = order ? order[b0 + blk] : blk + b0;
-  const uint32_t pbeg = blk * K, pend = pbeg + K < np ? pbeg + K : np;
-  const uint64_t us_b = pbeg + offsets[pbeg];
-  const uint32_t ntiles = btiles[blk];
-  const TileDesc *T = tiles + us_b / 16 + (uint64_t)(K + 2) * blk;
-  const uint64_t rbeg = eoff[pbeg] + (uint64_t)ENT_SPARE * blk, rend = eoff[pend] + (uint64_t)ENT_SPARE * (blk + 1);
-  const uint32_t elim = (uint32_t)(rend - rbeg) - ENT_SPARE;
+  blk = (uint32_t)__builtin_amdgcn_readfirstlane((int)blk);
+  if (blk >= b1) return;
+  const uint4 *bi = reinterpret_cast<const uint4 *>(btiles) + 2 * (size_t)blk;
+  const uint4 bi0 = bi[0], bi1 = bi[1];
+  const uint32_t pbeg = bi0.x, ntiles = bi0.y;
+  const uint64_t us_b = (uint64_t)bi1.x | (uint64_t)bi1.y << 32;
+  const TileDesc *T = tiles + us_b / 16 + pbeg + 2ull * blk;
+  const uint64_t rbeg = (uint64_t)bi1.z | (uint64_t)bi1.w << 32, rend = rbeg + bi0.z + ENT_SPARE;
+  const uint32_t elim = bi0.z;
 #ifdef GN_XCD_PROF
   const unsigned long long xp_t0 = __builtin_amdgcn_s_memrealtime();
 #endif
@@ -1270,7 +1279,9 @@
   const uint8_t *next_slot = K > 1 ? a.next_slot : nullptr;
   const int kc = K > 1 ? a.kc : 0;
   const int scr = K > 1 && a.kc;
-  const uint32_t nb = (uint32_t)((n + K - 1) / K), B0 = 0, B1 = nb;
+  if (!a.bfirst || !a.nblk || a.nblk > n) return hipErrorInvalidValue;
+  const uint32_t nb = a.nblk, B0 = 0, B1 = nb;
+  const uint32_t *xb = a.order ? a.xb : nullptr;
   const unsigned pg = (nb + PLAN_WAVES - 1) / PLAN_WAVES, g = a.swz == 1 ? 8 * ((nb + 7) / 8) : nb + nb / 16 + 8;
   auto stream_done = [&] {
     if (a.fin) (void)hipEventRecord(a.fin, s);
@@ -1284,7 +1295,7 @@
         if (e != hipSuccess) return e;
       }
       hipLaunchKernelGGL((plan_kernel<3072>), dim3(pg), dim3(GN_FRONT_WG), 0, s, net, a.parents, a.offsets, a.deltas,
-                         a.need_parent, a.need_child, next_slot, (uint32_t)n, K, B0, B1, kc, a.eoff, a.ent, a.tiles,
+                         a.need_parent, a.need_child, next_slot, a.bfirst, (uint32_t)n, K, B0, B1, kc, a.eoff, a.ent, a.tiles,
                          a.btiles, a.rows_out, a.pads_out, a.err, sliced ? a.pinfo : nullptr,
                          sliced ? ps::field_xu(3072, 3) : ps::field_xu(3072, 1), sliced ? ps::field_hu(3072, 3) : ps::field_hu(3072, 1));
       if (a.mid) (void)hipEventRecord(a.mid, s);
@@ -1292,7 +1303,7 @@
     if (!do_stream) {
     } else if (sliced) {
       for (int sl = 0; sl < 3; ++sl)
-        hipLaunchKernelGGL((stream_eval_kernel<3072, 3>), dim3(g), dim3(128), 0, s, net, a.offsets, (uint32_t)n, K, B0,
+        hipLaunchKernelGGL((stream_eval_kernel<3072, 3>), dim3(g), dim3(128), 0, s, net, a.offsets, a.bfirst, xb, (uint32_t)n, B0,
                            B1, a.swz, a.eoff, a.ent, a.tiles, a.btiles, a.order, a.out_parent, a.out_child, a.pool, scr,
                            a.err, a.pool + 64 + 8 * sl, sl, a.part, (uint64_t)a.npos, a.pinfo);
       stream_done();
@@ -1300,7 +1311,7 @@
         hipLaunchKernelGGL((slice_finish_kernel<3>), dim3((unsigned)((a.npos + 255) / 256)), dim3(256), 0, s, net,
                            a.part, a.pinfo, (uint64_t)a.npos, (uint32_t)n, a.out_parent, a.out_child);
     } else {
-      hipLaunchKernelGGL((stream_eval_kernel<3072>), dim3(g), dim3(384), 0, s, net, a.offsets, (uint32_t)n, K, B0, B1,
+      hipLaunchKernelGGL((stream_eval_kernel<3072>), dim3(g), dim3(384), 0, s, net, a.offsets, a.bfirst, xb, (uint32_t)n, B0, B1,
                          a.swz, a.eoff, a.ent, a.tiles, a.btiles, a.order, a.out_parent, a.out_child, a.pool, scr, a.err,
                          a.pool + 64, 0, nullptr, (uint64_t)0, nullptr);
       stream_done();
@@ -1308,12 +1319,12 @@
   } else if (net.L1 == 1024) {
     if (do_plan) {
       hipLaunchKernelGGL((plan_kernel<1024>), dim3(pg), dim3(GN_FRONT_WG), 0, s, net, a.parents, a.offsets, a.deltas,
-                         a.need_parent, a.need_child, next_slot, (uint32_t)n, K, B0, B1, kc, a.eoff, a.ent, a.tiles,
+                         a.need_parent, a.need_child, next_slot, a.bfirst, (uint32_t)n, K, B0, B1, kc, a.eoff, a.ent, a.tiles,
                          a.btiles, a.rows_out, a.pads_out, a.err, nullptr, ps::field_xu(1024, 1), ps::field_hu(1024, 1));
       if (a.mid) (void)hipEventRecord(a.mid, s);
     }
     if (do_stream) {
-      hipLaunchKernelGGL((stream_eval_kernel<1024>), dim3(g), dim3(128), 0, s, net, a.offsets, (uint32_t)n, K, B0, B1,
+      hipLaunchKernelGGL((stream_eval_kernel<1024>), dim3(g), dim3(128), 0, s, net, a.offsets, a.bfirst, xb, (uint32_t)n, B0, B1,
                          a.swz, a.eoff, a.ent, a.tiles, a.btiles, a.order, a.out_parent, a.out_child, a.pool, scr, a.err,
                          a.pool + 64, 0, nullptr, (uint64_t)0, nullptr);
       stream_done();
diff --git a/fishnet_amd/gpu_nnue.py b/fishnet_amd/gpu_nnue.py
--- a/fishnet_amd/gpu_nnue.py
+++ b/fishnet_amd/gpu_nnue.py
@@ -37,7 +37,8 @@
            "gn_random_games_uci"]
 OPT_INCREMENTAL_CHILDREN, OPT_XCD_SWIZZLE, OPT_KING_SORT, OPT_CHAIN, OPT_KING_CACHE = 1, 2, 3, 4, 5
 OPT_CHUNK_PARENTS, OPT_COALESCE, OPT_STREAM_SLICES, OPT_FAST_BATCH, OPT_EXPAND_PIPELINE = 6, 7, 8, 9, 10
-STAT_PLAN_NS, STAT_STREAM_NS, STAT_SCRATCH_PADS, STAT_FINISH_NS = 101, 102, 103, 104
+OPT_BLOCK_CUT = 11
+STAT_PLAN_NS, STAT_STREAM_NS, STAT_SCRATCH_PADS, STAT_FINISH_NS, STAT_BLOCKS = 101, 102, 103, 104, 105
 STAT_BATCH_LAUNCHES, STAT_BATCH_CALLS, STAT_FAST_BATCHES, STAT_FAST_FALLBACKS = 117, 118, 119, 120
 HOST_STAGES = {"parse": 110, "upload": 111, "replay": 112, "compute": 113, "download": 114, "tail": 115, "total": 116}
 EXPAND_STAGES = ["count_scan", "total_readback", "write_children", "classify", "small_net", "big_net", "finalize",
diff --git a/include/gpu_nnue.h b/include/gpu_nnue.h
--- a/include/gpu_nnue.h
+++ b/include/gpu_nnue.h
@@ -39,11 +39,13 @@
 #define GN_OPT_KING_SORT 3
 #define GN_OPT_KING_CACHE 5
 #define GN_OPT_CHAIN 4
+#define GN_OPT_BLOCK_CUT 11
 #define GN_OPT_STREAM_SLICES 8
 
 #define GN_STAT_PLAN_NS 101
 #define GN_STAT_STREAM_NS 102
 #define GN_STAT_FINISH_NS 104
+#define GN_STAT_BLOCKS 105
 #define GN_STAT_SCRATCH_PADS 103
 #define GN_STAT_HOST_PARSE_NS 110
 #define GN_STAT_HOST_UPLOAD_NS 111
diff --git a/rust/gpu-nnue-sys/src/lib.rs b/rust/gpu-nnue-sys/src/lib.rs
--- a/rust/gpu-nnue-sys/src/lib.rs
+++ b/rust/gpu-nnue-sys/src/lib.rs
@@ -28,10 +28,12 @@
 pub const GN_OPT_STREAM_SLICES: c_int = 8;
 pub const GN_OPT_FAST_BATCH: c_int = 9;
 pub const GN_OPT_EXPAND_PIPELINE: c_int = 10;
+pub const GN_OPT_BLOCK_CUT: c_int = 11;
 pub const GN_STAT_PLAN_NS: c_int = 101;
 pub const GN_STAT_STREAM_NS: c_int = 102;
 pub const GN_STAT_SCRATCH_PADS: c_int = 103;
 pub const GN_STAT_FINISH_NS: c_int = 104;
+pub const GN_STAT_BLOCKS: c_int = 105;
 pub const GN_STAT_HOST_PARSE_NS: c_int = 110;
 pub const GN_STAT_HOST_UPLOAD_NS: c_int = 111;
 pub const GN_STAT_HOST_REPLAY_NS: c_int = 112;
```

Measured after the change: 855.1 million (median of 2 runs). No clear change (-0.0%).
